# jshi31/T2ONet

Hardware: AMD Instinct MI355X
Metric: images/sec (train step: episode forward + END select + L1 + backward + gradient all-reduce + Adam, bs=64/GPU, 256x256 fp32) (higher is better)
Workload: dtype f32; 1 GPU; BASELINE.json configs[2]: full T2ONet episode/L1 train step (train_seq2seqL1.py:74-88), bs=64 per GPU, 256x256 fp32, FiveK-shaped synthetic batch, random-init weights; global_batch=64, parallelism=dp1: batch shards, one flat fp32 gradient all-reduce (22.2 M floats) per step, world_size=1

## Files before the change

include/t2onet_hip.h:

```cpp
#ifndef T2ONET_HIP_H
#define T2ONET_HIP_H

#include <stddef.h>

#ifdef __cplusplus
extern "C" {
#endif

#define T2O_OK 0
#define T2O_EINVAL 1
#define T2O_EUNSUPPORTED 2
#define T2O_EWORKSPACE 3
#define T2O_ELAUNCH 4

#define T2O_OP_IDENTITY (-1)
#define T2O_MAX_PARAM 24

int t2o_abi_version(void);
const char* t2o_last_error(void);
const char* t2o_source_digest(void);

int t2o_op_num_params(int op);

size_t t2o_workspace_bytes(int B, int H, int W);

int t2o_op_fwd(int op, const float* img, const float* param, int param_stride,
               const float* mask, int mask_ch, float* out, int B, int H, int W, void* stream);

int t2o_op_bwd(int op, const float* img, const float* param, int param_stride,
               const float* mask, int mask_ch, const float* gout,
               float* gimg, float* gparam, int gparam_stride,
               void* workspace, size_t workspace_bytes, int B, int H, int W, void* stream);

int t2o_apply_fwd(const int* op_id, const float* img, const float* param, int param_stride,
                  const float* mask, int mask_ch, float* out, int B, int H, int W, void* stream);
int t2o_apply_bwd(const int* op_id, const float* img, const float* param, int param_stride,
                  const float* mask, int mask_ch, const float* gout,
                  float* gimg, float* gparam, int gparam_stride,
                  void* workspace, size_t workspace_bytes, int B, int H, int W, void* stream);

int t2o_l1_fwd(const float* pred, const float* target, float* loss, size_t n,
               void* workspace, size_t workspace_bytes, void* stream);
int t2o_l1_bwd(const float* pred, const float* target, const float* gloss, float* gpred,
               size_t n, void* stream);

int t2o_end_select_l1_fwd(const float* const* imgs, int T, const long long* first, const float* target, float* loss, int B,
                          size_t row, void* workspace, size_t workspace_bytes, void* stream);
int t2o_end_select_l1_bwd(const float* const* imgs, float* const* gimgs, int T, const long long* first, const float* target,
                          const float* gloss, int B, size_t row, void* stream);

int t2o_op_fwd_l1(int op, const float* img, const float* param, int param_stride,
                  const float* mask, int mask_ch, const float* target, float* out, float* loss,
                  void* workspace, size_t workspace_bytes, int B, int H, int W, void* stream);
int t2o_op_bwd_l1(int op, const float* img, const float* param, int param_stride,
                  const float* mask, int mask_ch, const float* target, const float* gloss,
                  float* gimg, float* gparam, int gparam_stride,
                  void* workspace, size_t workspace_bytes, int B, int H, int W, void* stream);

int t2o_sequence_fwd(const int* ops, int K, const float* img, const float* params,
                     const float* target, float* acts, float* loss,
                     void* workspace, size_t workspace_bytes, int B, int H, int W, void* stream);
int t2o_sequence_bwd(const int* ops, int K, const float* img, const float* params,
                     const float* target, const float* acts, const float* gloss,
                     float* gimg, float* gparams, float* gbuf,
                     void* workspace, size_t workspace_bytes, int B, int H, int W, void* stream);

int t2o_fused_sequence_buffers(const int* ops, int K);
int t2o_fused_sequence_fwd(const int* ops, int K, const float* img, const float* params,
                           const float* target, float* out, float* loss, float* seg_bufs,
                           void* workspace, size_t workspace_bytes, int B, int H, int W, void* stream);
int t2o_fused_sequence_bwd(const int* ops, int K, const float* img, const float* params,
                           const float* target, const float* gloss, const float* gout,
                           float* gimg, float* gparams, const float* seg_bufs, float* gbuf,
                           void* workspace, size_t workspace_bytes, int B, int H, int W, void* stream);

int t2o_fused_sequence_l1_value_grad(const int* ops, int K, const float* img, const float* params,
                                     const float* target, const float* gloss, float* out, float* loss,
                                     float* gimg, float* gparams, float* seg_bufs, float* gbuf,
                                     void* workspace, size_t workspace_bytes, int B, int H, int W, void* stream);

int t2o_fused_sequence_prepare(const int* ops, int K);
int t2o_jit_set_cache_dir(const char* dir);
int t2o_jit_specialisations(void);

size_t t2o_candidates_workspace_bytes(int C, int H, int W);
int t2o_op_candidates_l1(int op, const float* img, const float* target, const float* params, int C,
                         int param_stride, float* loss, void* workspace, size_t workspace_bytes,
                         int H, int W, void* stream);

size_t t2o_candidates_multi_workspace_bytes(int J, int C, int H, int W);
int t2o_op_candidates_multi_l1(const int* ops, const int* img_index, int J, const float* imgs, int n_img,
                               const float* target, const float* params, int C, int param_stride, float* loss,
                               void* workspace, size_t workspace_bytes, int H, int W, void* stream);

size_t t2o_fit_multi_workspace_bytes(int J, int H, int W);
int t2o_fit_multi_l1_adam(const int* ops, const int* img_index, const int* target_index, int J, const float* imgs,
                          int n_img, const float* targets, int n_target, float* params, float* dist, void* workspace,
                          size_t workspace_bytes, int H, int W, int steps, double lr, double beta1, double beta2,
                          double eps, int check_every, double tol, void* stream);

size_t t2o_candidates_multi_masked_workspace_bytes(int J, int C, int H, int W);
int t2o_op_candidates_multi_l1_masked(const int* ops, const int* img_index, const int* mask_index, int J,
                                      const float* imgs, int n_img, const unsigned char* masks, int n_mask,
                                      const float* target, const float* params, int C, int param_stride, float* loss,
                                      void* workspace, size_t workspace_bytes, int H, int W, void* stream);
size_t t2o_fit_multi_masked_workspace_bytes(int J, int H, int W);
int t2o_fit_multi_l1_adam_masked(const int* ops, const int* img_index, const int* target_index, const int* mask_index,
                                 int J, const float* imgs, int n_img, const float* targets, int n_target,
                                 const unsigned char* masks, int n_mask, float* params, float* dist, void* workspace,
                                 size_t workspace_bytes, int H, int W, int steps, double lr, double beta1, double beta2,
                                 double eps, int check_every, double tol, void* stream);

size_t t2o_ssim_workspace_bytes(int B, int C, int H, int W);
int t2o_ssim_fwd(const float* img1, const float* img2, float* out,
                 void* workspace, size_t workspace_bytes, int B, int C, int H, int W, void* stream);
int t2o_ssim_bwd(const float* img1, const float* img2, const float* gout, float* g1, float* g2,
                 int B, int C, int H, int W, void* stream);

int t2o_attn_fwd(const float* q, const float* ctx, float* attn, float* mix,
                 int B, int L, int D, void* stream);
int t2o_attn_bwd(const float* q, const float* ctx, const float* attn, const float* gmix,
                 const float* gattn, float* gq, float* gctx, int B, int L, int D, void* stream);

int t2o_choose_op(const float* logp, float* op_mask, const float* u, float explore_prob, long long* pred_op, int* exec_op,
                  int B, int n_cls, void* stream);

size_t t2o_bn_workspace_bytes(int N, int C);
int t2o_bn_relu_fwd(const float* x, const float* res, const float* weight, const float* bias,
                    float* running_mean, float* running_var, float* save_mean, float* save_invstd, float* out,
                    float momentum, float eps, void* workspace, size_t workspace_bytes,
                    int N, int C, int HW, void* stream);
int t2o_bn_relu_bwd(const float* x, const float* y, const float* dy, const float* weight, const float* bias,
// ... 287 lines not shown
```

t2onet_amd/_lib.py:

```python
import ctypes
import os

import torch

_HERE = os.path.dirname(os.path.abspath(__file__))
LIB_PATH = os.path.join(_HERE, 'lib', 'libt2onet_hip.so')

c_f = ctypes.POINTER(ctypes.c_float)
c_i = ctypes.POINTER(ctypes.c_int)
_P = ctypes.c_void_p
_I = ctypes.c_int
_Z = ctypes.c_size_t
_F = ctypes.c_float
_D = ctypes.c_double

SIGNATURES = {
    't2o_abi_version': (_I, []),
    't2o_last_error': (ctypes.c_char_p, []),
    't2o_source_digest': (ctypes.c_char_p, []),
    't2o_op_num_params': (_I, [_I]),
    't2o_workspace_bytes': (_Z, [_I, _I, _I]),
    't2o_op_fwd': (_I, [_I, _P, _P, _I, _P, _I, _P, _I, _I, _I, _P]),
    't2o_op_bwd': (_I, [_I, _P, _P, _I, _P, _I, _P, _P, _P, _I, _P, _Z, _I, _I, _I, _P]),
    't2o_apply_fwd': (_I, [_P, _P, _P, _I, _P, _I, _P, _I, _I, _I, _P]),
    't2o_apply_bwd': (_I, [_P, _P, _P, _I, _P, _I, _P, _P, _P, _I, _P, _Z, _I, _I, _I, _P]),
    't2o_l1_fwd': (_I, [_P, _P, _P, _Z, _P, _Z, _P]),
    't2o_l1_bwd': (_I, [_P, _P, _P, _P, _Z, _P]),
    't2o_op_fwd_l1': (_I, [_I, _P, _P, _I, _P, _I, _P, _P, _P, _P, _Z, _I, _I, _I, _P]),
    't2o_op_bwd_l1': (_I, [_I, _P, _P, _I, _P, _I, _P, _P, _P, _P, _I, _P, _Z, _I, _I, _I, _P]),
    't2o_sequence_fwd': (_I, [_P, _I, _P, _P, _P, _P, _P, _P, _Z, _I, _I, _I, _P]),
    't2o_sequence_bwd': (_I, [_P, _I, _P, _P, _P, _P, _P, _P, _P, _P, _P, _Z, _I, _I, _I, _P]),
    't2o_fused_sequence_buffers': (_I, [_P, _I]),
    't2o_fused_sequence_fwd': (_I, [_P, _I, _P, _P, _P, _P, _P, _P, _P, _Z, _I, _I, _I, _P]),
    't2o_fused_sequence_bwd': (_I, [_P, _I, _P, _P, _P, _P, _P, _P, _P, _P, _P, _P, _Z, _I, _I, _I, _P]),
    't2o_fused_sequence_l1_value_grad': (_I, [_P, _I, _P, _P, _P, _P, _P, _P, _P, _P, _P, _P, _P, _Z, _I, _I, _I, _P]),
    't2o_candidates_workspace_bytes': (_Z, [_I, _I, _I]),
    't2o_op_candidates_l1': (_I, [_I, _P, _P, _P, _I, _I, _P, _P, _Z, _I, _I, _P]),
    't2o_candidates_multi_workspace_bytes': (_Z, [_I, _I, _I, _I]),
    't2o_op_candidates_multi_l1': (_I, [c_i, c_i, _I, _P, _I, _P, _P, _I, _I, _P, _P, _Z, _I, _I, _P]),
    't2o_fit_multi_workspace_bytes': (_Z, [_I, _I, _I]),
    't2o_fit_multi_l1_adam': (_I, [c_i, c_i, c_i, _I, _P, _I, _P, _I, _P, _P, _P, _Z, _I, _I, _I, _D, _D, _D, _D, _I, _D, _P]),
    't2o_candidates_multi_masked_workspace_bytes': (_Z, [_I, _I, _I, _I]),
    't2o_op_candidates_multi_l1_masked': (_I, [c_i, c_i, c_i, _I, _P, _I, _P, _I, _P, _P, _I, _I, _P, _P, _Z, _I, _I, _P]),
    't2o_fit_multi_masked_workspace_bytes': (_Z, [_I, _I, _I]),
    't2o_fit_multi_l1_adam_masked': (_I, [c_i, c_i, c_i, c_i, _I, _P, _I, _P, _I, _P, _I, _P, _P, _P, _Z, _I, _I, _I, _D, _D, _D, _D, _I,
                                          _D, _P]),
    't2o_ssim_workspace_bytes': (_Z, [_I, _I, _I, _I]),
    't2o_ssim_fwd': (_I, [_P, _P, _P, _P, _Z, _I, _I, _I, _I, _P]),
    't2o_ssim_bwd': (_I, [_P, _P, _P, _P, _P, _I, _I, _I, _I, _P]),
    't2o_wino_fused_wgrad_supported': (_I, [_I, _I, _I, _I, _I]),
    't2o_wino_fused_wgrad_workspace_bytes': (_Z, [_I, _I, _I, _I, _I]),
    't2o_wino_fused_wgrad_nhwc': (_I, [_P, _P, _P, _P, _P, _Z, _I, _I, _I, _I, _I, _I, _P]),
    't2o_comm_available': (_I, []),
    't2o_comm_unique_id': (_I, [_P]),
    't2o_comm_init_rank': (_I, [_P, _I, _P, _I]),
    't2o_comm_destroy': (_I, [_P]),
    't2o_allreduce': (_I, [_P, _Z, _P, _P]),
    't2o_allreduce_mean': (_I, [_P, _Z, _P, _P]),
    't2o_choose_op': (_I, [_P, _P, _P, _F, _P, _P, _I, _I, _P]),
    't2o_attn_fwd': (_I, [_P, _P, _P, _P, _I, _I, _I, _P]),
    't2o_attn_bwd': (_I, [_P, _P, _P, _P, _P, _P, _P, _I, _I, _I, _P]),
    't2o_bn_workspace_bytes': (_Z, [_I, _I]),
    't2o_bn_relu_fwd': (_I, [_P, _P, _P, _P, _P, _P, _P, _P, _P, _F, _F, _P, _Z, _I, _I, _I, _P]),
    't2o_bn_relu_bwd': (_I, [_P, _P, _P, _P, _P, _P, _P, _P, _P, _P, _P, _I, _P, _Z, _I, _I, _I, _P]),
    't2o_bn_nhwc_workspace_bytes': (_Z, [_I, _I]),
    't2o_bn_relu_nhwc_fwd': (_I, [_P, _P, _P, _P, _P, _P, _P, _P, _P, _F, _F, _I, _P, _Z, _I, _I, _P]),
    't2o_bn_relu_nhwc_bwd': (_I, [_P, _P, _P, _P, _P, _P, _P, _P, _P, _P, _P, _I, _I, _P, _Z, _I, _I, _P]),
    't2o_bn_relu_nhwc_fwd_partials': (_I, [_P, _P, _P, _P, _P, _P, _P, _P, _P, _F, _F, _I, _P, _I, _P, _Z, _I, _I, _P]),
    't2o_param_heads_fwd': (_I, [_P, _P, _P, _P, _P, _P, _P, _P, _P, _F, _F, _F, _F, _I, _I, _P]),
    't2o_param_heads_bwd': (_I, [_P, _P, _P, _P, _P, _P, _P, _P, _P, _P, _P, _P, _P, _P, _P, _F, _F, _F, _F, _I, _I, _P]),
    't2o_param_heads_bwd_acc': (_I, [_P, _P, _P, _P, _P, _P, _P, _P, _P, _P, _P, _P, _P, _P, _P, _F, _F, _F, _F, _I, _I, _I, _P]),
    't2o_adam_step': (_I, [_P, _P, _P, _P, _Z, _F, _F, _F, _F, _I, _P]),
    't2o_graph_memsets_to_kernels': (_I, [_P, _P]),
    't2o_conv3x3_wgrad_workspace_bytes': (_Z, [_I, _I, _I, _I, _I]),
    't2o_conv3x3_wgrad_nhwc': (_I, [_P, _P, _P, _P, _Z, _I, _I, _I, _I, _I, _P]),
    't2o_conv3x3_fwd_workspace_bytes': (_Z, [_I, _I, _I, _I, _I]),
    't2o_conv3x3_fwd_nhwc': (_I, [_P, _P, _P, _P, _Z, _I, _I, _I, _I, _I, _P]),
    't2o_conv3x3_dgrad_workspace_bytes': (_Z, [_I, _I, _I, _I, _I]),
    't2o_conv3x3_dgrad_nhwc': (_I, [_P, _P, _P, _P, _Z, _I, _I, _I, _I, _I, _P]),
    't2o_conv_set_zero_region': (_I, [_I, _P, _Z]),
    't2o_conv3x3s2_fwd_workspace_bytes': (_Z, [_I, _I, _I, _I, _I]),
    't2o_conv3x3s2_fwd_nhwc': (_I, [_P, _P, _P, _P, _Z, _I, _I, _I, _I, _I, _P]),
    't2o_conv3x3_fwd_stats_rows': (_I, [_I, _I, _I, _I, _I]),
    't2o_conv3x3_fwd_stats_nhwc': (_I, [_P, _P, _P, _P, _P, _Z, _I, _I, _I, _I, _I, _I, _P]),
    't2o_stem_fwd_stats_rows': (_I, [_I, _I, _I]),
    't2o_stem_fwd_nhwc': (_I, [_P, _P, _P, _P, _I, _I, _I, _I, _P]),
    't2o_stem_wgrad_workspace_bytes': (_Z, [_I, _I, _I, _I]),
    't2o_stem_wgrad_nhwc': (_I, [_P, _P, _P, _P, _Z, _I, _I, _I, _I, _P]),
    't2o_conv3x3s2_wgrad_workspace_bytes': (_Z, [_I, _I, _I, _I, _I]),
    't2o_conv3x3s2_wgrad_nhwc': (_I, [_P, _P, _P, _P, _Z, _I, _I, _I, _I, _I, _P]),
    't2o_conv3x3s2_dgrad_workspace_bytes': (_Z, [_I, _I, _I, _I, _I]),
    't2o_conv3x3s2_dgrad_nhwc': (_I, [_P, _P, _P, _P, _Z, _I, _I, _I, _I, _I, _P]),
    't2o_bn_relu_nhwc_bwd_acc': (_I, [_P, _P, _P, _P, _P, _P, _P, _P, _P, _P, _P, _I, _I, _I, _P, _Z, _I, _I, _P]),
    't2o_bn_relu_nhwc_bwd_partials_acc': (_I, [_P, _P, _P, _P, _P, _P, _P, _P, _P, _I, _I, _P, _I, _P, _Z, _I, _I, _P]),
    't2o_conv3x3_wgrad_acc_nhwc': (_I, [_P, _P, _P, _P, _Z, _I, _I, _I, _I, _I, _I, _I, _P]),
    't2o_conv_weight_transform': (_I, [_P, _P, _I, _I, _I, _I, _P]),
    't2o_conv_weight_transform_batch': (_I, [_P, _P, _P, _P, _P, _P, _I, _P]),
    't2o_wino_weight_transform_batch': (_I, [_P, _P, _P, _P, _I, _P]),
    't2o_wino_weight_transform_chunked_batch': (_I, [_P, _P, _P, _P, _I, _P]),
    't2o_end_select_l1_fwd': (_I, [_P, _I, _P, _P, _P, _I, _Z, _P, _Z, _P]),
    't2o_end_select_l1_bwd': (_I, [_P, _P, _I, _P, _P, _P, _I, _Z, _P]),
    't2o_wino_padded_tiles': (_I, [_I, _I, _I]),
    't2o_wino_weight_transform': (_I, [_P, _P, _I, _I, _P]),
    't2o_gemm_nt_batched': (_I, [_P, _P, _P, _I, _I, _I, _I, _I, _P]),
    't2o_gemm': (_I, [_P, _P, _P, _I, _I, _I, _I, _I, _I, _I, _I, _I, _P]),
    't2o_colsum': (_I, [_P, _P, _I, _I, _I, _I, _P]),
    't2o_gemm_tn_splits': (_I, [_I, _I, _I, _I]),
    't2o_gemm_tn_batched': (_I, [_P, _P, _P, _I, _I, _I, _I, _I, _P]),
    't2o_gemm_tn_batched_ld': (_I, [_P, _P, _P, _I, _I, _I, _I, _I, _I, _I, _P]),
    't2o_wino_input_transform': (_I, [_P, _P, _I, _I, _I, _I, _P]),
    't2o_wino_input_transform_ld': (_I, [_P, _P, _I, _I, _I, _I, _I, _P]),
    't2o_wino_stats_rows': (_I, [_I, _I, _I, _I]),
    't2o_wino_output_transform': (_I, [_P, _P, _P, _P, _I, _I, _I, _I, _P]),
    't2o_wino_dy_transform': (_I, [_P, _P, _I, _I, _I, _I, _P]),
    't2o_wino_dy_transforms': (_I, [_P, _P, _P, _I, _I, _I, _I, _P]),
    't2o_wino_dy_transforms_ld': (_I, [_P, _P, _P, _I, _I, _I, _I, _I, _P]),
    't2o_wino_dy_transform_ld': (_I, [_P, _P, _I, _I, _I, _I, _I, _P]),
    't2o_wino_dw_transform': (_I, [_P, _P, _I, _I, _I, _I, _P]),
    't2o_conv3x3_dgrad_pre_nhwc': (_I, [_P, _P, _P, _P, _P, _Z, _I, _I, _I, _I, _I, _P]),
    't2o_conv3x3_dgrad_bnsums_rows': (_I, [_I, _I, _I, _I, _I]),
    't2o_wino_fused_supported': (_I, [_I, _I, _I, _I, _I]),
    't2o_wino_fused_stats_rows': (_I, [_I, _I, _I]),
    't2o_wino_u_chunked': (_I, [_P, _P, _I, _I, _P]),
    't2o_wino_fused_conv_nhwc': (_I, [_P, _P, _P, _P, _P, _P, _I, _I, _I, _I, _I, _P]),
    't2o_wino_fused_conv_bnsums_nhwc': (_I, [_P, _P, _P, _P, _P, _P, _P, _P, _P, _P, _I, _I, _I, _I, _I, _P]),
    't2o_conv3x3_dgrad_pre_bnsums_nhwc': (_I, [_P, _P, _P, _P, _P, _P, _P, _P, _P, _P, _Z, _I, _I, _I, _I, _I, _P]),
    't2o_conv3x3s2_dgrad_pre_nhwc': (_I, [_P, _P, _P, _P, _Z, _I, _I, _I, _I, _I, _P]),
    't2o_stem_fwd': (_I, [_P, _P, _P, _P, _I, _I, _I, _I, _I, _P]),
    't2o_stem_fwd_any': (_I, [_P, _P, _P, _P, _I, _I, _I, _I, _I, _P]),
    't2o_stem_wgrad': (_I, [_P, _P, _P, _P, _Z, _I, _I, _I, _I, _I, _I, _P]),
    't2o_stem_dgrad': (_I, [_P, _P, _P, _I, _I, _I, _I, _I, _I, _P]),
    't2o_conv1x1s2_fwd_nhwc': (_I, [_P, _P, _P, _I, _I, _I, _I, _I, _P]),
    't2o_conv1x1s2_dgrad_acc_nhwc': (_I, [_P, _P, _P, _I, _I, _I, _I, _I, _P]),
    't2o_conv1x1s2_wgrad_workspace_bytes': (_Z, [_I, _I, _I, _I, _I]),
    't2o_conv1x1s2_wgrad_nhwc': (_I, [_P, _P, _P, _P, _Z, _I, _I, _I, _I, _I, _I, _P]),
    't2o_fused_sequence_prepare': (_I, [_P, _I]),
    't2o_jit_set_cache_dir': (_I, [ctypes.c_char_p]),
    't2o_jit_specialisations': (_I, []),
    't2o_conv3x3_any_fwd_nhwc': (_I, [_P, _P, _P, _I, _I, _I, _I, _I, _I, _P]),
    't2o_conv3x3_any_dgrad_nhwc': (_I, [_P, _P, _P, _P, _I, _I, _I, _I, _I, _I, _P]),
    't2o_conv3x3_any_wgrad_workspace_bytes': (_Z, [_I, _I, _I, _I, _I, _I]),
    't2o_conv3x3_any_wgrad_nhwc': (_I, [_P, _P, _P, _P, _Z, _I, _I, _I, _I, _I, _I, _I, _P]),
    't2o_lstm_layer_fwd': (_I, [_P, _P, _P, _P, _P, _P, _P, _P, _P, _I, _I, _I, _I, _P]),
    't2o_lstm_layer_bwd': (_I, [_P, _P, _P, _P, _P, _P, _P, _P, _P, _P, _I, _I, _I, _I, _P]),
    't2o_bn_dual_nhwc_workspace_bytes': (_Z, [_I, _I]),
    't2o_bn_dual_relu_nhwc_fwd': (_I, [_P, _P, _I, _P] + [_P] * 13 + [_F, _F, _F, _F, _P, _Z, _I, _I, _P]),
    't2o_bn_dual_relu_nhwc_bwd_acc': (_I, [_P] * 18 + [_I, _P, _Z, _I, _I, _P]),
    't2o_image_feature_fwd': (_I, [_P, _P]),
    't2o_image_feature_bwd': (_I, [_P, _P]),
    't2o_decoder_step_fwd': (_I, [_P, _P]),
    't2o_decoder_step_bwd': (_I, [_P, _P]),
    't2o_resize_u8_to_f32': (_I, [_P, _P, _I, _I, _I, _P, _P]),
    't2o_f32_to_u8_hwc': (_I, [_P, _I, _I, _I, _P, _P]),
    't2o_replay_u8': (_I, [_P, _P, _P, _I, _P, _P]),
    't2o_replay_u8_masked': (_I, [_P, _P, _P, _P, _I, _P, _P, _P, _I, _P]),
    't2o_feather_weights': (_I, [_D, _P, _P]),
    't2o_feather_workspace_bytes': (_Z, [_P, _I]),
    't2o_feather_u8': (_I, [_P, _P, _P, _I, _P, _Z, _P]),
    't2o_eval_metrics_workspace_bytes': (_Z, [_I, _I, _I, _I]),
    't2o_eval_metrics': (_I, [_P, _P, _I, _P, _P, _P, _I, _P, _Z, _I, _I, _I, _I, _P]),
    't2o_end_select_var_mean_workspace_bytes': (_Z, [_Z]),
    't2o_end_select_var_mean': (_I, [_P, _P, _I, _I, _I, _Z, _P, _P, _Z, _P]),
    't2o_rle_union_u8': (_I, [_P, _P, _I, _I, _I, ctypes.c_longlong, _P, ctypes.c_longlong, _P]),
    't2o_mask_select': (_I, [_P, _P, _P, _P, _I, _I, _I, _I, _I, _P]),
}


class ImageFeatureArgs(ctypes.Structure):
    _fields_ = ([(n, _P) for n in ('fc_w', 'fc_b', 'bn_w', 'bn_b', 'running_mean', 'running_var', 'num_batches_tracked', 'pooled',
                                   'pooled_copy', 'fc_out', 'stats', 'feat', 'g_feat', 'd_fc', 'd_bn', 'd_pooled')]
                + [('momentum', _F), ('eps', _F), ('training', _I), ('B', _I), ('K', _I), ('D', _I)])


class DecoderStepArgs(ctypes.Structure):
    _fields_ = ([(n, _P) for n in ('emb', 'vis_w', 'vis_b', 'w_ih0', 'w_hh0', 'b_ih0', 'b_hh0', 'w_ih1', 'w_hh1', 'b_ih1', 'b_hh1',
                                   'lo_w', 'lo_b', 'out_w', 'out_b', 'prev_op', 'feat', 'h0', 'c0', 'h1', 'c1', 'enc', 'step_in',
                                   'feat_copy', 'hp0', 'hp1', 'prev_op_copy', 'gates0', 'gates1', 'h0n', 'c0n', 'h1n', 'c1n', 'attn', 'mix', 'ctx', 'logp',
                                   'g_logp', 'g_ctx', 'g_h0n', 'g_c0n', 'g_h1n', 'g_c1n', 'd_logits', 'd_lin', 'd_gates1',
                                   'd_gates0', 'd_step_in', 'd_vis', 'd_ctx', 'd_mix', 'd_qa', 'd_q', 'd_x1', 'd_feat', 'd_h0',
                                   'd_c0', 'd_h1', 'd_c1', 'd_enc')]
                + [(n, _I) for n in ('B', 'L', 'D', 'E', 'V')])

_lib = None

# ... 42 lines not shown
```

t2onet_amd/csrc/t2o_block_programs.h:

```cpp
#pragma once
#ifndef __HIPCC_RTC__
#include <stddef.h>
#include <stdint.h>
#endif

#include "t2o_pixel_math.h"

namespace t2o {

constexpr int kThreads = 256;
constexpr int kRedSlots = 24;

constexpr int kTileW = 64;
constexpr int kTileH = 16;
constexpr int kStripRows = 4;
constexpr int kStripWideCols = 248;
T2O_HD int strip_bwd_segments(int W) { return W <= 256 ? 1 : (W + kStripWideCols - 1) / kStripWideCols; }
constexpr int kFwdStripRows = 2;
constexpr int kRowStride = 72;
constexpr int kIntOff = 4;

struct OpArgs {
  const float* img;
  const float* param;
  const float* mask;
  const int* op_id;
  const float* gout;
  const float* target;
  const float* gloss;
  float* out;
  float* gimg;
  float* partials;
  float* loss_partials;
  int op;
  int param_stride;
  int mask_ch;
  int B, H, W;
  int iters;
  int nblk_max;
  float inv_n;
};

T2O_HD size_t plane_off(const OpArgs& a, int b, int c) { return ((size_t)b * 3 + c) * (size_t)a.H * a.W; }

T2O_HD float mask_at(const OpArgs& a, int b, int c, size_t px) {
  const int mc = a.mask_ch == 3 ? c : 0;
  return a.mask[((size_t)b * a.mask_ch + mc) * (size_t)a.H * a.W + px];
}

template <int V>
T2O_HD void load_vec(const float* p, float (&r)[V]) {
#if defined(__HIP_DEVICE_COMPILE__)
  if constexpr (V == 4) {
    const float4 t = *reinterpret_cast<const float4*>(p);
    r[0] = t.x; r[1] = t.y; r[2] = t.z; r[3] = t.w;
    return;
  }
#endif
  T2O_UNROLL
  for (int i = 0; i < V; ++i) r[i] = p[i];
}

template <int V>
T2O_HD void store_vec(float* p, const float (&r)[V]) {
#if defined(__HIP_DEVICE_COMPILE__)
  if constexpr (V == 4) {
    *reinterpret_cast<float4*>(p) = make_float4(r[0], r[1], r[2], r[3]);
    return;
  }
#endif
  T2O_UNROLL
  for (int i = 0; i < V; ++i) p[i] = r[i];
}

T2O_HD float sign_of(float d) { return d > 0.0f ? 1.0f : (d < 0.0f ? -1.0f : 0.0f); }

constexpr int kTabStride = 64;
constexpr int kTabK = 0, kTabP = 24, kTabSum = 51, kTabScale = 54, kTabRsum = 57;

T2O_HD void curve_table_build(const float* p, bool color, float* t) {
  for (int c = 0; c < 3; ++c) {
    const float* row = color ? p + c * kCurveSteps : p;
    float s = 0.0f, run = 0.0f;
    for (int i = 0; i < kCurveSteps; ++i) {
      t[kTabK + c * kCurveSteps + i] = row[i];
      t[kTabP + c * (kCurveSteps + 1) + i] = run;
      run = run + (1.0f / kCurveSteps) * row[i];
      s = s + row[i];
    }
    t[kTabP + c * (kCurveSteps + 1) + kCurveSteps] = run;
    s = s + 1e-10f;
    t[kTabSum + c] = s;
    t[kTabRsum + c] = 1.0f / s;
    t[kTabScale + c] = t[kTabRsum + c] * (float)kCurveSteps;
  }
}

T2O_HD void curve_locate(float x, int& i, float& frac, bool unit = false) {
  const float x8 = unit ? fminf(x * (float)kCurveSteps, (float)kCurveSteps - 0.5f)
                        : fminf(fmaxf(x * (float)kCurveSteps, 0.0f), (float)kCurveSteps - 0.5f);
  i = (int)x8;
  const float d = x - (float)i / kCurveSteps;
  frac = unit ? d : fminf(fmaxf(d, 0.0f), 1.0f / kCurveSteps);
}

T2O_HD float curve_lut_fwd(const float* t, bool color, int c, float x, bool unit = false) {
  const int cc = color ? c : 0;
  int i; float frac;
  curve_locate(x, i, frac, unit);
  const float total = t[kTabP + cc * (kCurveSteps + 1) + i] + frac * t[kTabK + cc * kCurveSteps + i];
  return color ? total * t[kTabScale + cc]
               : div_by(total * (float)kCurveSteps, t[kTabSum + cc], t[kTabRsum + cc]);
}

T2O_HD float curve_lut_bwd_1(const float* t, bool color, int c, float x, float g, float* red_row, bool first = false,
                             bool unit = false) {
  const int cc = color ? c : 0;
  const float* kk = t + kTabK + cc * kCurveSteps;
  int i; float frac;
  curve_locate(x, i, frac, unit);
  const float d = x - (float)i / kCurveSteps;
  float slope = (unit || (d >= 0.0f && d <= 1.0f / kCurveSteps)) ? kk[i] : 0.0f;
  if (d == 0.0f && i > 0) slope += kk[i - 1];
  curve_bins_accumulate(x, g, red_row, first);
  return g * t[kTabScale + cc] * slope;
}

struct SampleView {
  const float* x;
  const float* g;
  const float* m;
  float* o;
  const float* t;
  unsigned hw;
  unsigned mstride;
};

template <int V, bool MASKED, bool L1>
T2O_HD float pointwise_fwd_thread(const OpArgs& a, int op, int b, int blk, int tid) {
  const unsigned hw = (unsigned)a.H * (unsigned)a.W;
  const unsigned groups = hw / V;
  const size_t sb = (size_t)b * 3 * hw;
  SampleView s;
  s.x = a.img + sb;
  s.o = a.out + sb;
  s.t = L1 ? a.target + sb : nullptr;
  s.m = MASKED ? a.mask + (size_t)b * a.mask_ch * hw : nullptr;
  s.mstride = (MASKED && a.mask_ch == 3) ? hw : 0u;
  const float* prow = a.param ? a.param + (size_t)b * a.param_stride : nullptr;
  Curve cv;
  if (op == OP_COLOR || op == OP_TONE) curve_load(cv, prow, op == OP_COLOR);
  float p0[1] = {(op >= 0 && prow) ? prow[0] : 0.0f};
  float l1 = 0.0f;
  for (int it = 0; it < a.iters; ++it) {
    const unsigned g = ((unsigned)blk * a.iters + it) * kThreads + tid;
    if (g >= groups) break;
    const unsigned px = g * V;
    float x[3][V], o[3][V], mk[3][V];
    T2O_UNROLL
    for (int c = 0; c < 3; ++c) {
      load_vec<V>(s.x + c * hw + px, x[c]);
      if (MASKED && (c == 0 || s.mstride)) load_vec<V>(s.m + c * s.mstride + px, mk[c]);
    }
    T2O_UNROLL
    for (int i = 0; i < V; ++i) {
      Rgb xi = {{x[0][i], x[1][i], x[2][i]}};
      if (op == OP_IDENTITY) {
        o[0][i] = xi.c[0]; o[1][i] = xi.c[1]; o[2][i] = xi.c[2];
      } else {
        const Rgb r = pointwise_fwd(op, xi, p0, cv);
        T2O_UNROLL
        for (int c = 0; c < 3; ++c) {
          float z = r.c[c];
          if (MASKED) z = blend(z, xi.c[c], s.mstride ? mk[c][i] : mk[0][i]);
          o[c][i] = clamp01(z);
        }
      }
    }
    T2O_UNROLL
    for (int c = 0; c < 3; ++c) store_vec<V>(s.o + c * hw + px, o[c]);
    if (L1) {
      T2O_UNROLL
      for (int c = 0; c < 3; ++c) {
        float t[V];
        load_vec<V>(s.t + c * hw + px, t);
        T2O_UNROLL
        for (int i = 0; i < V; ++i) l1 += fabsf(o[c][i] - t[i]);
      }
    }
  }
  return l1;
}

template <int V, bool MASKED, bool L1>
T2O_HD void pointwise_bwd_thread(const OpArgs& a, int op, int b, int blk, int tid, float (&red)[kRedSlots], const float* tab) {
  const unsigned hw = (unsigned)a.H * (unsigned)a.W;
  const unsigned groups = hw / V;
  const size_t sb = (size_t)b * 3 * hw;
  SampleView s;
  s.x = a.img + sb;
  s.g = (L1 ? a.target : a.gout) + sb;
  s.o = a.gimg ? a.gimg + sb : nullptr;
  s.m = MASKED ? a.mask + (size_t)b * a.mask_ch * hw : nullptr;
  s.mstride = (MASKED && a.mask_ch == 3) ? hw : 0u;
  const float* prow = a.param ? a.param + (size_t)b * a.param_stride : nullptr;
  Curve cv;
  float p0[1] = {(op >= 0 && prow) ? prow[0] : 0.0f};
  const float gs = L1 ? a.gloss[0] * a.inv_n : 0.0f;
  for (int it = 0; it < a.iters; ++it) {
    const unsigned g = ((unsigned)blk * a.iters + it) * kThreads + tid;
    if (g >= groups) break;
    const unsigned px = g * V;
    float x[3][V], gg[3][V], gx[3][V], mk[3][V];
    T2O_UNROLL
    for (int c = 0; c < 3; ++c) {
      load_vec<V>(s.x + c * hw + px, x[c]);
      load_vec<V>(s.g + c * hw + px, gg[c]);
      if (MASKED && (c == 0 || s.mstride)) load_vec<V>(s.m + c * s.mstride + px, mk[c]);
    }
    if (op == OP_TONE || op == OP_COLOR) {
      const bool color = op == OP_COLOR;
      float dep = 0.0f;
      T2O_UNROLL
      for (int i = 0; i < V; ++i) {
        T2O_UNROLL
        for (int c = 0; c < 3; ++c) {
          const float xv = T2O_CHAIN(x[c][i], dep);
          const float r = curve_lut_fwd(tab, color, c, xv);
          const float m = MASKED ? (s.mstride ? mk[c][i] : mk[0][i]) : 1.0f;
          const float z = MASKED ? blend(r, xv, m) : r;
          const float gz = L1 ? sign_of(clamp01(z) - gg[c][i]) * gs : gg[c][i];
          const float dz = (z >= 0.0f && z <= 1.0f) ? gz : 0.0f;
          const int kc = color ? c : 0;
          const float gi = curve_lut_bwd_1(tab, color, c, xv, MASKED ? dz * m : dz, red + kc * kCurveSteps);
          gx[c][i] = MASKED ? gi + dz * (1.0f - m) : gi;
          dep = gx[c][i];
          T2O_UNROLL
          for (int j = 0; j < kCurveSteps; ++j) T2O_KEEP(red[kc * kCurveSteps + j]);
        }
      }
    } else {
    T2O_UNROLL
    for (int i = 0; i < V; ++i) {
      Rgb xi = {{x[0][i], x[1][i], x[2][i]}};
      if (op == OP_IDENTITY) {
        T2O_UNROLL
        for (int c = 0; c < 3; ++c) gx[c][i] = L1 ? sign_of(xi.c[c] - gg[c][i]) * gs : gg[c][i];
        continue;
      }
      Rgb go, gpass;
      if (!MASKED && !L1 && !clamp_can_act(op, xi)) {
        go.c[0] = gg[0][i]; go.c[1] = gg[1][i]; go.c[2] = gg[2][i];
        const Rgb gi = pointwise_bwd(op, xi, p0, cv, go, red);
        T2O_UNROLL
        for (int c = 0; c < 3; ++c) gx[c][i] = gi.c[c];
        continue;
      }
      const Rgb r = pointwise_fwd(op, xi, p0, cv);
      T2O_UNROLL
      for (int c = 0; c < 3; ++c) {
        const float m = MASKED ? (s.mstride ? mk[c][i] : mk[0][i]) : 1.0f;
        const float z = MASKED ? blend(r.c[c], xi.c[c], m) : r.c[c];
        const float gz = L1 ? sign_of(clamp01(z) - gg[c][i]) * gs : gg[c][i];
        const float dz = (z >= 0.0f && z <= 1.0f) ? gz : 0.0f;
        go.c[c] = MASKED ? dz * m : dz;
        gpass.c[c] = MASKED ? dz * (1.0f - m) : 0.0f;
      }
      const Rgb gi = pointwise_bwd(op, xi, p0, cv, go, red);
      T2O_UNROLL
      for (int c = 0; c < 3; ++c) gx[c][i] = gi.c[c] + gpass.c[c];
    }
    }
    if (s.o) {
      T2O_UNROLL
      for (int c = 0; c < 3; ++c) store_vec<V>(s.o + c * hw + px, gx[c]);
    }
  }
}

T2O_HD int tile_rows(int halo) { return kTileH + 2 * halo; }
T2O_HD int tile_floats(int halo) { return tile_rows(halo) * kRowStride; }

template <int V, int HALO>
T2O_HD void tile_load(const float* src, unsigned hw, int planes, int H, int W, int y0, int x0, float* lds, int tid) {
  constexpr int rows = kTileH + 2 * HALO;
  constexpr int plane_floats = rows * kRowStride;
  if (V == 4) {
    constexpr int per_plane = rows * (kTileW / 4);
    for (int i = tid; i < planes * per_plane; i += kThreads) {
      const int c = i / per_plane, rem = i % per_plane;
      const int r = rem / (kTileW / 4), q = rem % (kTileW / 4);
      const int gy = y0 - HALO + r, gx = x0 + 4 * q;
      float v[4] = {0.0f, 0.0f, 0.0f, 0.0f};
      if (gy >= 0 && gy < H && gx < W) load_vec<4>(src + ((unsigned)c * hw + (unsigned)gy * (unsigned)W + (unsigned)gx), v);
      store_vec<4>(lds + c * plane_floats + r * kRowStride + kIntOff + 4 * q, v);
    }
    constexpr int hper = rows * 2 * HALO;
    for (int i = tid; i < planes * hper; i += kThreads) {
      const int c = i / hper, rem = i % hper;
      const int r = rem / (2 * HALO), k = rem % (2 * HALO);
      const int j = k < HALO ? k - HALO : kTileW + (k - HALO);
      const int gy = y0 - HALO + r, gx = x0 + j;
      float v = 0.0f;
      if (gy >= 0 && gy < H && gx >= 0 && gx < W) v = src[(unsigned)c * hw + (unsigned)gy * (unsigned)W + (unsigned)gx];
      lds[c * plane_floats + r * kRowStride + kIntOff + j] = v;
    }
  } else {
    constexpr int cols = kTileW + 2 * HALO;
    constexpr int per_plane = rows * cols;
    for (int i = tid; i < planes * per_plane; i += kThreads) {
      const int c = i / per_plane, rem = i % per_plane;
      const int r = rem / cols, j = rem % cols - HALO;
      const int gy = y0 - HALO + r, gx = x0 + j;
      float v = 0.0f;
      if (gy >= 0 && gy < H && gx >= 0 && gx < W) v = src[(unsigned)c * hw + (unsigned)gy * (unsigned)W + (unsigned)gx];
      lds[c * plane_floats + r * kRowStride + kIntOff + j] = v;
    }
  }
}

T2O_HD float tile_at(const float* lds, int halo, int c, int r, int j) {
  return lds[c * tile_floats(halo) + (r + halo) * kRowStride + kIntOff + j];
}

T2O_HD void tile_origin(const OpArgs& a, int tile, int& y0, int& x0) {
  const int tiles_x = (a.W + kTileW - 1) / kTileW;
  y0 = (tile / tiles_x) * kTileH;
  x0 = (tile % tiles_x) * kTileW;
}
T2O_HD int sharp_num_tiles(int H, int W) {
  return ((W + kTileW - 1) / kTileW) * ((H + kTileH - 1) / kTileH);
}

T2O_HD int sharp_fwd_lds_floats() { return 3 * tile_floats(1); }

template <int V>
T2O_HD void sharp_fwd_phase_load(const OpArgs& a, int b, int tile, int tid, float* lds) {
  int y0, x0;
  tile_origin(a, tile, y0, x0);
  tile_load<V, 1>(a.img + plane_off(a, b, 0), (unsigned)a.H * (unsigned)a.W, 3, a.H, a.W, y0, x0, lds, tid);
}

T2O_HD void tile_quad(const float* lds, int halo, int c, int r, int j, float (&q)[4]) {
  load_vec<4>(lds + c * tile_floats(halo) + (r + halo) * kRowStride + kIntOff + j, q);
}

struct Sides { float L, R; };
T2O_HD Sides quad_sides(const float* lds, int halo, int c, int r, int j0, const float (&ce)[4]) {
  Sides s;
#if defined(__HIP_DEVICE_COMPILE__)
  const float l = __builtin_bit_cast(float, __builtin_amdgcn_update_dpp(0, __builtin_bit_cast(int, ce[3]), 0x111, 0xF, 0xF, true));
  const float rr = __builtin_bit_cast(float, __builtin_amdgcn_update_dpp(0, __builtin_bit_cast(int, ce[0]), 0x101, 0xF, 0xF, true));
  const float e = tile_at(lds, halo, c, r, j0 == 0 ? -1 : kTileW);
  s.L = j0 == 0 ? e : l;
  s.R = j0 == kTileW - 4 ? e : rr;
#else
// ... 95 lines not shown
      const bool in = n == 4 ? quad_in : (row_in && x0 + j0 + i >= 0 && x0 + j0 + i < a.W);
      const float left = i == 0 ? L : ce[i > 0 ? i - 1 : 0], right = i == n - 1 ? R : ce[i < 3 ? i + 1 : 3];
      const float d = sharp_delta(ce[i], up[i], left, right, dn[i]);
      const float m = a.mask_ch ? mq[i] : 1.0f;
      float z = ce[i] + p * d;
      if (a.mask_ch) z = blend(z, ce[i], m);
      const float gz = a.target ? sign_of(clamp01(z) - gq[i]) * gs : gq[i];
      dz[i] = (in && z >= 0.0f && z <= 1.0f) ? gz : 0.0f;
      if (interior) red0 += dz[i] * m * d;
    }
  }
  float* dst = G + c * tile_floats(1) + (r + 1) * kRowStride + kIntOff + j0;
  if (n == 4) store_vec<4>(dst, dz); else dst[0] = dz[0];
}

template <int V>
T2O_HD void sharp_bwd_phase_dz(const OpArgs& a, int b, int tile, int tid, float* lds, float& red0) {
  int y0, x0;
  tile_origin(a, tile, y0, x0);
  const float p = a.param[(size_t)b * a.param_stride];
  const float gs = a.target ? a.gloss[0] * a.inv_n : 0.0f;
  const int rows = kTileH + 2;
  if (V == 4) {
    const int per = rows * (kTileW / 4);
    for (int i = tid; i < 3 * per; i += kThreads) {
      const int c = i / per, rem = i % per;
      sharp_dz_quad(a, p, gs, y0, x0, c, rem / (kTileW / 4) - 1, 4 * (rem % (kTileW / 4)), 4, lds, red0);
    }
    for (int i = tid; i < 3 * rows * 2; i += kThreads) {
      const int c = i / (rows * 2), rem = i % (rows * 2);
      sharp_dz_quad(a, p, gs, y0, x0, c, rem / 2 - 1, (rem % 2) ? kTileW : -1, 1, lds, red0);
    }
  } else {
    const int cols = kTileW + 2, per = rows * cols;
    for (int i = tid; i < 3 * per; i += kThreads) {
      const int c = i / per, rem = i % per;
      sharp_dz_quad(a, p, gs, y0, x0, c, rem / cols - 1, rem % cols - 1, 1, lds, red0);
    }
  }
}

template <int V>
T2O_HD void sharp_bwd_phase_out(const OpArgs& a, int b, int tile, int tid, const float* lds) {
  int y0, x0;
  tile_origin(a, tile, y0, x0);
  const int ty = tid / (kTileW / 4), tx = tid % (kTileW / 4);
  const int gy = y0 + ty, gx0 = x0 + 4 * tx;
  const bool live = gy < a.H && gx0 < a.W && a.gimg;
  const float p = a.param[(size_t)b * a.param_stride];
  const float* G = lds + sharp_bwd_g_off();
  const float* M = lds + sharp_bwd_m_off();
  T2O_UNROLL
  for (int c = 0; c < 3; ++c) {
    const int mc = a.mask_ch == 3 ? c : 0;
    float up[4], ce[4], dn[4], o[4], pass[4];
    tile_quad(G, 1, c, ty - 1, 4 * tx, up);
    tile_quad(G, 1, c, ty, 4 * tx, ce);
    tile_quad(G, 1, c, ty + 1, 4 * tx, dn);
    const Sides sg = quad_sides(G, 1, c, ty, 4 * tx, ce);
    float L = sg.L, R = sg.R;
    T2O_UNROLL
    for (int i = 0; i < 4; ++i) pass[i] = 0.0f;
    if (a.mask_ch) {
      float mu[4], mcq[4], md[4];
      tile_quad(M, 1, mc, ty - 1, 4 * tx, mu);
      tile_quad(M, 1, mc, ty, 4 * tx, mcq);
      tile_quad(M, 1, mc, ty + 1, 4 * tx, md);
      const Sides sm = quad_sides(M, 1, mc, ty, 4 * tx, mcq);
      L *= sm.L;
      R *= sm.R;
      T2O_UNROLL
      for (int i = 0; i < 4; ++i) {
        pass[i] = ce[i] * (1.0f - mcq[i]);
        up[i] *= mu[i]; ce[i] *= mcq[i]; dn[i] *= md[i];
      }
    }
    T2O_UNROLL
    for (int i = 0; i < 4; ++i) {
      const float left = i == 0 ? L : ce[i > 0 ? i - 1 : 0], right = i == 3 ? R : ce[i < 3 ? i + 1 : 3];
      o[i] = pass[i] + (ce[i] + p * sharp_delta(ce[i], up[i], left, right, dn[i]));
    }
    if (!live) continue;
    float* dst = a.gimg + plane_off(a, b, c) + (size_t)gy * a.W + gx0;
    if (V == 4) store_vec<4>(dst, o);
    else for (int i = 0; i < 4 && gx0 + i < a.W; ++i) dst[i] = o[i];
  }
}

constexpr int kMaxChain = 8;
constexpr int kAccStride = 65;

struct ChainArgs {
  const float* img;
  const float* params;
  const float* gout;
  const float* target;
  const float* gloss;
  float* out;
  float* gimg;
  float* partials;
  float* loss_partials;
  int ops[kMaxChain];
  int src[kMaxChain];
  int slot_off[kMaxChain + 1];
  int bin_off[kMaxChain + 1];
  int K, B, H, W, iters, nblk;
  int param_stride, gparam_stride;
  float inv_n;
};

T2O_HD bool is_curve(int op) { return op == OP_COLOR || op == OP_TONE; }

T2O_HD void chain_build_table(const ChainArgs& a, int b, int k, float* tab) {
  float* t = tab + k * kTabStride;
  const float* p = a.params + ((size_t)a.src[k] * a.B + b) * a.param_stride;
  const int op = a.ops[k];
  if (!is_curve(op)) { t[0] = p[0]; return; }
  curve_table_build(p, op == OP_COLOR, t);
}

T2O_HD Rgb chain_op_fwd(int op, const Rgb& x, const float* t, bool unit = false) {
  Rgb o;
  switch (op) {
    case OP_BRIGHTNESS: return brightness_fwd(x, t[0]);
    case OP_CONTRAST:   return contrast_fwd(x, t[0]);
    case OP_SATURATION: return saturation_fwd(x, t[0]);
    case OP_COLOR:
    case OP_TONE:
      T2O_UNROLL
      for (int c = 0; c < 3; ++c) o.c[c] = curve_lut_fwd(t, op == OP_COLOR, c, x.c[c], unit);
      return o;
    case OP_WHITE: o.c[0] = o.c[1] = o.c[2] = 1.0f; return o;
    default: return x;
  }
}

template <bool COLOR>
T2O_HD Rgb chain_curve_bwd(const Rgb& x, const float* t, const Rgb& dz, float* red, bool first, bool unit = false) {
  Rgb gx;
  T2O_UNROLL
  for (int c = 0; c < 3; ++c) {
    constexpr int kOne = COLOR ? 1 : 0;
    const int cc = c * kOne;
    gx.c[c] = curve_lut_bwd_1(t, COLOR, c, x.c[c], dz.c[c], red + cc * kCurveSteps, first && (COLOR || c == 0), unit);
  }
  return gx;
}

T2O_HD float chain_slot_value(const ChainArgs& a, int s, const float* bsum) { return bsum[s]; }

T2O_HD Rgb chain_scalar_bwd(int op, const Rgb& x, const float* t, const Rgb& dz, float* red) {
  Curve unused;
  float p0[1] = {t[0]};
  return pointwise_bwd(op, x, p0, unused, dz, red);
}

template <int V, bool L1>
T2O_HD float chain_fwd_thread(const ChainArgs& a, int b, int blk, int tid, const float* tab) {
  const unsigned hw = (unsigned)a.H * (unsigned)a.W;
  const unsigned groups = hw / V;
  const size_t sb = (size_t)b * 3 * hw;
  const float* xin = a.img + sb;
  float* o = a.out + sb;
  float l1 = 0.0f;
  for (int it = 0; it < a.iters; ++it) {
    const unsigned g = ((unsigned)blk * a.iters + it) * kThreads + tid;
// ... 692 lines not shown
```

t2onet_amd/csrc/t2o_kernels.hip:

```cpp
#include <hip/hip_runtime.h>
#include <stdio.h>
#include <stdlib.h>
#include <string.h>

#include <type_traits>

#include "../../include/t2onet_hip.h"
#include "t2o_block_programs.h"
#include "t2o_chain_kernels.h"
#include "t2o_jit.h"

using namespace t2o;

namespace {

thread_local char g_err[256] = "";

int fail(int code, const char* msg) {
  snprintf(g_err, sizeof(g_err), "%s", msg);
  return code;
}

}
namespace t2o { int set_error(int code, const char* msg) { return fail(code, msg); } }
namespace {

template <int OP, int V, bool MASKED, bool L1>
__global__ __launch_bounds__(kThreads) void k_point_fwd(OpArgs a, int nblk) {
  int b, blk;
  wg_coords(nblk, b, blk);
  const int op = (OP == OP_DYNAMIC) ? a.op_id[b] : OP;
  if (OP == OP_DYNAMIC && op == OP_SHARPNESS) return;
  float l1 = 0.0f;
  if (OP == OP_DYNAMIC) {
    switch (op) {
#define T2O_CASE(K) case K: l1 = pointwise_fwd_thread<V, MASKED, L1>(a, K, b, blk, threadIdx.x); break;
      T2O_CASE(OP_BRIGHTNESS) T2O_CASE(OP_CONTRAST) T2O_CASE(OP_SATURATION) T2O_CASE(OP_COLOR)
      T2O_CASE(OP_TONE) T2O_CASE(OP_WHITE)
#undef T2O_CASE
      default: l1 = pointwise_fwd_thread<V, MASKED, L1>(a, OP_IDENTITY, b, blk, threadIdx.x); break;
    }
  } else {
    l1 = pointwise_fwd_thread<V, MASKED, L1>(a, OP, b, blk, threadIdx.x);
  }
  if (L1) block_reduce_store1(l1, a.loss_partials + (size_t)b * a.nblk_max + blk);
}

template <int OP, int V, bool MASKED, bool L1>
__global__ __launch_bounds__(kThreads) void k_point_bwd(OpArgs a, int nblk) {
  int b, blk;
  wg_coords(nblk, b, blk);
  const int op = (OP == OP_DYNAMIC) ? a.op_id[b] : OP;
  if (OP == OP_DYNAMIC && op == OP_SHARPNESS) return;
  float red[kRedSlots];
#pragma unroll
  for (int i = 0; i < kRedSlots; ++i) red[i] = 0.0f;
  __shared__ float tab[kTabStride];
  if (OP == OP_COLOR || OP == OP_TONE || OP == OP_DYNAMIC) {
    if ((op == OP_COLOR || op == OP_TONE) && threadIdx.x == 0)
      curve_table_build(a.param + (size_t)b * a.param_stride, op == OP_COLOR, tab);
    __syncthreads();
  }
  if (OP == OP_DYNAMIC) {
    switch (op) {
#define T2O_CASE(K) case K: pointwise_bwd_thread<V, MASKED, L1>(a, K, b, blk, threadIdx.x, red, tab); break;
      T2O_CASE(OP_BRIGHTNESS) T2O_CASE(OP_CONTRAST) T2O_CASE(OP_SATURATION) T2O_CASE(OP_COLOR)
      T2O_CASE(OP_TONE) T2O_CASE(OP_WHITE)
#undef T2O_CASE
      default: pointwise_bwd_thread<V, MASKED, L1>(a, OP_IDENTITY, b, blk, threadIdx.x, red, tab); break;
    }
  } else {
    pointwise_bwd_thread<V, MASKED, L1>(a, OP, b, blk, threadIdx.x, red, tab);
  }
  if (op == OP_IDENTITY || op == OP_WHITE) return;
  block_reduce_store(red, nred_of(op), a.partials + ((size_t)b * a.nblk_max + blk) * kRedSlots);
}

template <bool DYN, int V>
__global__ __launch_bounds__(kThreads) void k_sharp_fwd(OpArgs a, int tiles) {
  extern __shared__ __attribute__((aligned(16))) float lds[];
  int b, tile;
  wg_coords(tiles, b, tile);
  if (DYN && a.op_id[b] != OP_SHARPNESS) return;
  sharp_fwd_phase_load<V>(a, b, tile, threadIdx.x, lds);
  __syncthreads();
  const float l1 = sharp_fwd_phase_compute<V>(a, b, tile, threadIdx.x, lds);
  if (a.target) block_reduce_store1(l1, a.loss_partials + (size_t)b * a.nblk_max + tile);
}


__device__ __forceinline__ float dpp_wave_shr1(float v) {
  return __builtin_bit_cast(float, __builtin_amdgcn_update_dpp(0, __builtin_bit_cast(int, v), 0x138, 0xF, 0xF, true));
}
__device__ __forceinline__ float dpp_wave_shl1(float v) {
  return __builtin_bit_cast(float, __builtin_amdgcn_update_dpp(0, __builtin_bit_cast(int, v), 0x130, 0xF, 0xF, true));
}

template <bool DYN, bool WIDE, int ROWS>
__global__ __launch_bounds__(kThreads) void k_sharp_fwd_strip(OpArgs a, int nblk, int nseg) {
  int b, blk;
  wg_coords(nblk, b, blk);
  if (DYN && a.op_id[b] != OP_SHARPNESS) return;
  const int lane = threadIdx.x & 63, wave = threadIdx.x >> 6;
  const int y0 = (blk / nseg) * (4 * ROWS) + wave * ROWS, gx0 = (blk % nseg) * 256 + 4 * lane;
  const bool col_live = gx0 < a.W;
  const unsigned hw = (unsigned)a.H * (unsigned)a.W;
  const float p = a.param[(size_t)b * a.param_stride];
  const bool ext_l = WIDE && lane == 0 && gx0 > 0 && col_live, ext_r = WIDE && lane == 63 && gx0 + 4 < a.W;
  float l1 = 0.0f;
#pragma unroll 1
  for (int c = 0; c < 3; ++c) {
    const float* xp = a.img + ((size_t)b * 3 + c) * hw;
    float xr[ROWS + 2][4], tg[ROWS][4];
#pragma unroll
    for (int k = 0; k < ROWS + 2; ++k) {
      const int y = y0 - 1 + k;
      xr[k][0] = xr[k][1] = xr[k][2] = xr[k][3] = 0.0f;
      if (col_live && y >= 0 && y < a.H) load_vec<4>(xp + (unsigned)y * (unsigned)a.W + (unsigned)gx0, xr[k]);
    }
    if (a.target) {
#pragma unroll
      for (int k = 0; k < ROWS; ++k) {
        const int y = y0 + k;
        tg[k][0] = tg[k][1] = tg[k][2] = tg[k][3] = 0.0f;
        if (col_live && y < a.H) load_vec<4>(a.target + ((size_t)b * 3 + c) * hw + (unsigned)y * (unsigned)a.W + (unsigned)gx0, tg[k]);
      }
    }
#pragma unroll
    for (int k = 0; k < ROWS; ++k) {
      const int y = y0 + k;
      const bool live = col_live && y < a.H;
      const float* ce = xr[k + 1];
      float L = dpp_wave_shr1(ce[3]), R = dpp_wave_shl1(ce[0]);
      if (ext_l && live) L = xp[(unsigned)y * (unsigned)a.W + (unsigned)gx0 - 1];
      if (ext_r && live) R = xp[(unsigned)y * (unsigned)a.W + (unsigned)gx0 + 4];
      float o[4];
#pragma unroll
      for (int i = 0; i < 4; ++i) {
        const float left = i == 0 ? L : ce[i > 0 ? i - 1 : 0], right = i == 3 ? R : ce[i < 3 ? i + 1 : 3];
        o[i] = ce[i] + p * sharp_delta(ce[i], xr[k][i], left, right, xr[k + 2][i]);
      }
      if (!live) continue;
      const unsigned off = (unsigned)y * (unsigned)a.W + (unsigned)gx0;
      if (a.mask_ch) {
        float m[4];
        load_vec<4>(a.mask + ((size_t)b * a.mask_ch + (a.mask_ch == 3 ? c : 0)) * hw + off, m);
#pragma unroll
        for (int i = 0; i < 4; ++i) o[i] = blend(o[i], ce[i], m[i]);
      }
#pragma unroll
      for (int i = 0; i < 4; ++i) o[i] = clamp01(o[i]);
      store_vec<4>(a.out + ((size_t)b * 3 + c) * hw + off, o);
      if (a.target) {
#pragma unroll
        for (int i = 0; i < 4; ++i) l1 += fabsf(o[i] - tg[k][i]);
      }
    }
  }
  if (a.target) block_reduce_store1(l1, a.loss_partials + (size_t)b * a.nblk_max + blk);
}


template <bool DYN, bool WIDE, bool MASKED, bool VAL = false>
__global__ __launch_bounds__(kThreads) void k_sharp_bwd_strip(OpArgs a, int nblk, int nseg) {
  int b, blk;
  wg_coords(nblk, b, blk);
  if (DYN && a.op_id[b] != OP_SHARPNESS) return;
  const int lane = threadIdx.x & 63, wave = threadIdx.x >> 6;
  const int y0 = (blk / nseg) * (4 * kStripRows) + wave * kStripRows;
  const int gx0 = WIDE ? (blk % nseg) * kStripWideCols - 4 + 4 * lane : 4 * lane;
  const bool col_live = gx0 >= 0 && gx0 < a.W;
  const bool own = !WIDE || (lane >= 1 && lane <= 62);
  const unsigned hw = (unsigned)a.H * (unsigned)a.W;
  const float p = a.param[(size_t)b * a.param_stride];
  const float gs = a.target ? a.gloss[0] * a.inv_n : 0.0f;
  float red0 = 0.0f;
  float l1 = 0.0f;
#pragma unroll 1
  for (int c = 0; c < 3; ++c) {
    const float* xp = a.img + ((size_t)b * 3 + c) * hw;
    const float* gp = (a.target ? a.target : a.gout) + ((size_t)b * 3 + c) * hw;
    const float* mp = MASKED ? a.mask + ((size_t)b * a.mask_ch + (a.mask_ch == 3 ? c : 0)) * hw : nullptr;
    float xr[kStripRows + 4][4], g[kStripRows + 2][4], mk[MASKED ? kStripRows + 2 : 1][4], pass[MASKED ? kStripRows : 1][4];
#pragma unroll
    for (int k = 0; k < kStripRows + 4; ++k) {
      const int y = y0 - 2 + k;
      xr[k][0] = xr[k][1] = xr[k][2] = xr[k][3] = 0.0f;
      if (col_live && y >= 0 && y < a.H) load_vec<4>(xp + (unsigned)y * (unsigned)a.W + (unsigned)gx0, xr[k]);
    }
#pragma unroll
    for (int k = 0; k < kStripRows + 2; ++k) {
      const int y = y0 - 1 + k;
      g[k][0] = g[k][1] = g[k][2] = g[k][3] = 0.0f;
      if (MASKED) mk[k][0] = mk[k][1] = mk[k][2] = mk[k][3] = 0.0f;
      if (col_live && y >= 0 && y < a.H) {
        load_vec<4>(gp + (unsigned)y * (unsigned)a.W + (unsigned)gx0, g[k]);
        if (MASKED) load_vec<4>(mp + (unsigned)y * (unsigned)a.W + (unsigned)gx0, mk[k]);
      }
    }
#pragma unroll
    for (int k = 0; k < kStripRows + 2; ++k) {
      const int y = y0 - 1 + k;
      const bool in = col_live && y >= 0 && y < a.H;
      const float* ce = xr[k + 1];
      const float L = dpp_wave_shr1(ce[3]), R = dpp_wave_shl1(ce[0]);
      const bool mine = VAL && k >= 1 && k <= kStripRows && own && in;
      float oz[VAL ? 4 : 1];
#pragma unroll
      for (int i = 0; i < 4; ++i) {
        const float left = i == 0 ? L : ce[i > 0 ? i - 1 : 0], right = i == 3 ? R : ce[i < 3 ? i + 1 : 3];
        const float d = sharp_delta(ce[i], xr[k][i], left, right, xr[k + 2][i]);
        const float m = MASKED ? mk[k][i] : 1.0f;
        float z = ce[i] + p * d;
        if (MASKED) z = blend(z, ce[i], m);
        if constexpr (VAL) {
          oz[i] = clamp01(z);
          if (mine) l1 += fabsf(oz[i] - g[k][i]);
        }
        const float gz = a.target ? sign_of(clamp01(z) - g[k][i]) * gs : g[k][i];
        const float dz = (in && z >= 0.0f && z <= 1.0f) ? gz : 0.0f;
        g[k][i] = MASKED ? dz * m : dz;
        if (MASKED && k >= 1 && k <= kStripRows) pass[k - 1][i] = dz * (1.0f - m);
        if (k >= 1 && k <= kStripRows && own) red0 += dz * m * d;
      }
      if constexpr (VAL) {
        if (a.out && mine) store_vec<4>(a.out + ((size_t)b * 3 + c) * hw + (unsigned)y * (unsigned)a.W + (unsigned)gx0, oz);
      }
    }
#pragma unroll
    for (int k = 1; k <= kStripRows; ++k) {
      const int y = y0 - 1 + k;
      const float* ce = g[k];
      const float L = dpp_wave_shr1(ce[3]), R = dpp_wave_shl1(ce[0]);
      float o[4];
#pragma unroll
      for (int i = 0; i < 4; ++i) {
        const float left = i == 0 ? L : ce[i > 0 ? i - 1 : 0], right = i == 3 ? R : ce[i < 3 ? i + 1 : 3];
        o[i] = ce[i] + p * sharp_delta(ce[i], g[k - 1][i], left, right, g[k + 1][i]);
        if (MASKED) o[i] = pass[k - 1][i] + o[i];
      }
      if (a.gimg && own && col_live && y < a.H)
        store_vec<4>(a.gimg + ((size_t)b * 3 + c) * hw + (unsigned)y * (unsigned)a.W + (unsigned)gx0, o);
    }
  }
  block_reduce_store1(red0, a.partials + ((size_t)b * a.nblk_max + blk) * kRedSlots);
  if constexpr (VAL) {
    __syncthreads();
    block_reduce_store1(l1, a.loss_partials + (size_t)b * a.nblk_max + blk);
  }
}

template <bool DYN, int V>
__global__ __launch_bounds__(kThreads) void k_sharp_bwd(OpArgs a, int tiles) {
  extern __shared__ __attribute__((aligned(16))) float lds[];
  int b, tile;
  wg_coords(tiles, b, tile);
  if (DYN && a.op_id[b] != OP_SHARPNESS) return;
  sharp_bwd_phase_load<V>(a, b, tile, threadIdx.x, lds);
  __syncthreads();
  float red0 = 0.0f;
  sharp_bwd_phase_dz<V>(a, b, tile, threadIdx.x, lds, red0);
  __syncthreads();
  sharp_bwd_phase_out<V>(a, b, tile, threadIdx.x, lds);
  block_reduce_store1(red0, a.partials + ((size_t)b * a.nblk_max + tile) * kRedSlots);
}

template <int V, bool L1>
__global__ __launch_bounds__(kThreads) void k_chain_fwd(ChainArgs a) {
  __shared__ float tab[kMaxChain * kTabStride];
  int b, blk;
  wg_coords(a.nblk, b, blk);
  if ((int)threadIdx.x < a.K) chain_build_table(a, b, threadIdx.x, tab);
  __syncthreads();
  const float l1 = chain_fwd_thread<V, L1>(a, b, blk, threadIdx.x, tab);
  if (L1) block_reduce_store1(l1, a.loss_partials + (size_t)b * a.nblk + blk);
}

template <int V, bool L1, class SEQ>
__global__ __launch_bounds__(kThreads) void k_chain_fwd_static(ChainArgs a) { chain_fwd_static_body<V, L1, SEQ>(a); }

template <int V, bool L1>
__global__ __launch_bounds__(kThreads) void k_chain_bwd(ChainArgs a) {
  extern __shared__ __attribute__((aligned(16))) float lds[];
  __shared__ float tab[kMaxChain * kTabStride];
  __shared__ float bsum[kMaxChainBins];
  int b, blk;
  wg_coords(a.nblk, b, blk);
  const int S = a.slot_off[kMaxChain], NB = a.bin_off[kMaxChain];
  for (int i = threadIdx.x; i < NB * kAccStride; i += kThreads) lds[i] = 0.0f;
  if ((int)threadIdx.x < a.K) chain_build_table(a, b, threadIdx.x, tab);
  __syncthreads();
  LdsAcc acc{lds};
  const float l1 = chain_bwd_thread<V, L1>(a, b, blk, threadIdx.x, tab, lds + NB * kAccStride, acc);
  if (L1 && a.loss_partials) block_reduce_store1(l1, a.loss_partials + (size_t)b * a.nblk + blk);
  __syncthreads();
  for (int s = threadIdx.x; s < NB; s += kThreads) {
    float sum = 0.0f;
    for (int q = 0; q < kThreads / 4; ++q) sum += lds[s * kAccStride + q];
    bsum[s] = sum;
  }
  __syncthreads();
  for (int s = threadIdx.x; s < S; s += kThreads)
    a.partials[((size_t)b * a.nblk + blk) * S + s] = chain_slot_value(a, s, bsum);
}

template <bool L1, class SEQ, bool SV_LDS, int MINW, bool VAL = false>
__global__ __launch_bounds__(kThreads, MINW) void k_chain_bwd_static(ChainArgs a) { chain_bwd_static_body<L1, SEQ, SV_LDS, VAL>(a); }

__global__ __launch_bounds__(kThreads) void k_chain_finalize(ChainArgs a, float* gparams) {
  __shared__ float part[8][kMaxChainSlots];
  __shared__ float sums[kMaxChainSlots];
  const int b = blockIdx.x;
  const int S = a.slot_off[kMaxChain];
  for (int w = threadIdx.x; w < S * 8; w += kThreads) {
    const int s = w % S, lane8 = w / S;
    float acc = 0.0f;
    for (int k = lane8; k < a.nblk; k += 8) acc += a.partials[((size_t)b * a.nblk + k) * S + s];
    part[lane8][s] = acc;
  }
  __syncthreads();
  for (int s = threadIdx.x; s < S; s += kThreads) {
    float v = 0.0f;
#pragma unroll
    for (int j = 0; j < 8; ++j) v += part[j][s];
    sums[s] = v;
// ... 120 lines not shown
  for (int it = 0; it < iters; ++it) {
    const size_t g = ((size_t)blockIdx.x * iters + it) * kThreads + threadIdx.x;
    if (g * V >= n) break;
    float p[V], t[V];
    load_vec<V>(pred + g * V, p);
    load_vec<V>(target + g * V, t);
#pragma unroll
    for (int i = 0; i < V; ++i) acc += fabsf(p[i] - t[i]);
  }
  block_reduce_store1(acc, partial + blockIdx.x);
}

__global__ __launch_bounds__(kThreads) void k_l1_finalize(const float* partial, int nblk, float inv_n, float* loss) {
  float acc = 0.0f;
  for (int k = threadIdx.x; k < nblk; k += kThreads) acc += partial[k];
  __shared__ float out1;
  block_reduce_store1(acc, &out1);
  __syncthreads();
  if (threadIdx.x == 0) loss[0] = out1 * inv_n;
}

template <int V>
__global__ __launch_bounds__(kThreads) void k_l1_bwd(const float* pred, const float* target, const float* gloss,
                                                     float* gpred, size_t n, float inv_n, int iters) {
  const float gs = gloss[0] * inv_n;
  for (int it = 0; it < iters; ++it) {
    const size_t g = ((size_t)blockIdx.x * iters + it) * kThreads + threadIdx.x;
    if (g * V >= n) break;
    float p[V], t[V], o[V];
    load_vec<V>(pred + g * V, p);
    load_vec<V>(target + g * V, t);
#pragma unroll
    for (int i = 0; i < V; ++i) o[i] = sign_of(p[i] - t[i]) * gs;
    store_vec<V>(gpred + g * V, o);
  }
}

struct EndSelArgs {
  const float* img[8];
  float* gimg[8];
  int T;
};

__device__ __forceinline__ const float* end_sel_src(const EndSelArgs& s, int f) {
  const float* p = s.img[0];
#pragma unroll
  for (int t = 1; t < 8; ++t) p = (f == t) ? s.img[t] : p;
  return p;
}

template <int V>
__global__ __launch_bounds__(kThreads) void k_end_l1_fwd(EndSelArgs s, const long long* first, const float* target, float* partial,
                                                         size_t n, size_t row, int iters) {
  float acc = 0.0f;
  for (int it = 0; it < iters; ++it) {
    const size_t g = ((size_t)blockIdx.x * iters + it) * kThreads + threadIdx.x;
    if (g * V >= n) break;
    const int f = (int)first[(g * V) / row];
    float p[V], t[V];
    load_vec<V>(end_sel_src(s, f) + g * V, p);
    load_vec<V>(target + g * V, t);
#pragma unroll
    for (int i = 0; i < V; ++i) acc += fabsf(p[i] - t[i]);
  }
  block_reduce_store1(acc, partial + blockIdx.x);
}

template <int V>
__global__ __launch_bounds__(kThreads) void k_end_l1_bwd(EndSelArgs s, const long long* first, const float* target, const float* gloss,
                                                         size_t n, size_t row, float inv_n, int iters) {
  const float gs = gloss[0] * inv_n;
  for (int it = 0; it < iters; ++it) {
    const size_t g = ((size_t)blockIdx.x * iters + it) * kThreads + threadIdx.x;
    if (g * V >= n) break;
    const int f = (int)first[(g * V) / row];
    float p[V], t[V], o[V], z[V];
    load_vec<V>(end_sel_src(s, f) + g * V, p);
    load_vec<V>(target + g * V, t);
#pragma unroll
    for (int i = 0; i < V; ++i) { o[i] = sign_of(p[i] - t[i]) * gs; z[i] = 0.0f; }
#pragma unroll
    for (int k = 0; k < 8; ++k)
      if (k < s.T) store_vec<V>(s.gimg[k] + g * V, f == k ? o : z);
  }
}

__global__ __launch_bounds__(kThreads) void k_ssim_fwd(SsimArgs s) {
  extern __shared__ __attribute__((aligned(16))) float lds[];
  int plane, tile;
  wg_coords(s.tiles, plane, tile);
  ssim_phase_load(s, plane, tile, threadIdx.x, lds);
  __syncthreads();
  ssim_phase_rows(s, threadIdx.x, lds);
  __syncthreads();
  const float v = ssim_phase_cols(s, tile, threadIdx.x, lds);
  block_reduce_store1(v, s.partials + (size_t)plane * s.tiles + tile);
}

__global__ __launch_bounds__(kThreads) void k_ssim_finalize(const float* partials, int per_sample, float inv, float* out) {
  float acc = 0.0f;
  for (int k = threadIdx.x; k < per_sample; k += kThreads) acc += partials[(size_t)blockIdx.x * per_sample + k];
  __shared__ float out1;
  block_reduce_store1(acc, &out1);
  __syncthreads();
  if (threadIdx.x == 0) out[blockIdx.x] = out1 * inv;
}

__global__ __launch_bounds__(kThreads) void k_ssim_bwd(SsimBwdArgs s) {
  __shared__ __attribute__((aligned(16))) float lds[kSsimBD + 4 * kSsimBMid * kSsimBMidStride];
  int plane, tile;
  wg_coords(s.tiles, plane, tile);
  ssim_bwd_phase_load(s, plane, tile, threadIdx.x, lds);
  __syncthreads();
  ssim_bwd_phase_rows(s, threadIdx.x, lds);
  __syncthreads();
  ssim_bwd_phase_deriv(s, plane, tile, threadIdx.x, lds);
  __syncthreads();
  ssim_bwd_phase_drows(s, threadIdx.x, lds);
  __syncthreads();
  ssim_bwd_phase_out(s, plane, tile, threadIdx.x, lds);
}

__global__ __launch_bounds__(kThreads) void k_candidates_l1(CandArgs a) {
  __shared__ float tab[kCandPerBlock * kTabStride];
  __shared__ float wsum[kCandPerBlock][kThreads / 64];
  const int blk = blockIdx.x % a.nblk, group = blockIdx.x / a.nblk;
  const int c0 = group * kCandPerBlock;
  if ((int)threadIdx.x < kCandPerBlock && c0 + (int)threadIdx.x < a.C)
    cand_build_table(a, c0 + threadIdx.x, tab + threadIdx.x * kTabStride);
  float x[3][kCandPix], tg[3][kCandPix];
  const int npx = cand_load(a, blk, threadIdx.x, x, tg);
  __syncthreads();
  for (int j = 0; j < kCandPerBlock; ++j) {
    if (c0 + j >= a.C) break;
    const float s = wave_sum(cand_eval(a, tab + j * kTabStride, x, tg, npx));
    if ((threadIdx.x & 63) == 0) wsum[j][threadIdx.x >> 6] = s;
  }
  __syncthreads();
  if ((int)threadIdx.x < kCandPerBlock && c0 + (int)threadIdx.x < a.C) {
    const int j = threadIdx.x;
    a.partials[(size_t)(c0 + j) * a.nblk + blk] = ((wsum[j][0] + wsum[j][1]) + wsum[j][2]) + wsum[j][3];
  }
}

constexpr int kMaxCandJobs = 64;
struct MultiCandArgs {
  const float* imgs;
  const float* target;
  const float* params;
  float* partials;
  int op[kMaxCandJobs];
  int img_index[kMaxCandJobs];
  int C, param_stride, H, W, nblk;
};

struct MultiCandMaskArgs : MultiCandArgs {
  const unsigned char* masks;
  int mask_index[kMaxCandJobs];
};

template <bool MASKED>
__global__ __launch_bounds__(kThreads) void k_candidates_multi_l1(typename std::conditional<MASKED, MultiCandMaskArgs, MultiCandArgs>::type m) {
  __shared__ float tab[kCandPerBlock * kTabStride];
  __shared__ float wsum[kCandPerBlock][kThreads / 64];
  const int job = blockIdx.y;
  CandArgs a;
// ... 244 lines not shown
  const float* cb = ctx + (size_t)b * L * D;
  const float* gm = gmix + (size_t)b * D;
  for (int l = wave; l < L; l += kThreads / 64) {
    float part = 0.0f;
    for (int e = lane; e < D; e += 64) part += gm[e] * cb[(size_t)l * D + e];
    const float s = wave_sum(part);
    if (lane == 0) ga[l] = s + (gattn ? gattn[(size_t)b * L + l] : 0.0f);
  }
  if ((int)threadIdx.x < L) pr[threadIdx.x] = attn[(size_t)b * L + threadIdx.x];
  __syncthreads();
  float dot = 0.0f;
  for (int l = 0; l < L; ++l) dot += pr[l] * ga[l];
  if ((int)threadIdx.x < L) gs[threadIdx.x] = pr[threadIdx.x] * (ga[threadIdx.x] - dot);
  __syncthreads();
  for (int e = threadIdx.x; e < D; e += kThreads) {
    const float qe = qb[e], ge = gm[e];
    float acc = 0.0f;
    for (int l = 0; l < L; ++l) {
      acc += gs[l] * cb[(size_t)l * D + e];
      gctx[((size_t)b * L + l) * D + e] = pr[l] * ge + gs[l] * qe;
    }
    gq[(size_t)b * D + e] = acc;
  }
}

int env_int(const char* name, int dflt) {
  const char* s = getenv(name);
  return s ? atoi(s) : dflt;
}

Geometry launch_geometry(int B, int H, int W) {
  constexpr int forced = 0;
  return t2o::geometry(B, H, W, forced);
}

size_t ws_block_rows(const Geometry& g, int B, int H, int W) {
  int vec, iters, nblk;
  chain_geometry(B, H, W, 0, vec, iters, nblk, 1);
  return (size_t)(g.nblk_max > nblk ? g.nblk_max : nblk);
}
size_t ws_partials_floats(const Geometry& g, int B, int H, int W) { return (size_t)B * ws_block_rows(g, B, H, W) * kMaxChainSlots; }
size_t ws_loss_floats(const Geometry& g, int B, int H, int W) { return (size_t)B * ws_block_rows(g, B, H, W); }

int check_launch(const char* what) {
  const hipError_t e = hipGetLastError();
  if (e != hipSuccess) {
    snprintf(g_err, sizeof(g_err), "%s: %s", what, hipGetErrorString(e));
    return T2O_ELAUNCH;
  }
  return T2O_OK;
}

bool op_supported(int op) { return op == OP_IDENTITY || (op >= 0 && op <= 7 && op != OP_INPAINT); }

#define T2O_POINT_OPS(KERNEL, V, M, L)                                                        \
  switch (op) {                                                                             \
    case OP_IDENTITY:   KERNEL<OP_IDENTITY, V, M, L><<<grid, kThreads, 0, st>>>(a, nblk); break;   \
    case OP_BRIGHTNESS: KERNEL<OP_BRIGHTNESS, V, M, L><<<grid, kThreads, 0, st>>>(a, nblk); break; \
    case OP_CONTRAST:   KERNEL<OP_CONTRAST, V, M, L><<<grid, kThreads, 0, st>>>(a, nblk); break;   \
    case OP_SATURATION: KERNEL<OP_SATURATION, V, M, L><<<grid, kThreads, 0, st>>>(a, nblk); break; \
    case OP_COLOR:      KERNEL<OP_COLOR, V, M, L><<<grid, kThreads, 0, st>>>(a, nblk); break;      \
    case OP_TONE:       KERNEL<OP_TONE, V, M, L><<<grid, kThreads, 0, st>>>(a, nblk); break;       \
    case OP_WHITE:      KERNEL<OP_WHITE, V, M, L><<<grid, kThreads, 0, st>>>(a, nblk); break;      \
    case OP_DYNAMIC:    KERNEL<OP_DYNAMIC, V, M, L><<<grid, kThreads, 0, st>>>(a, nblk); break;    \
    default: break;                                                                         \
  }
#define T2O_POINT_CASES(KERNEL, V)                                    \
  if (masked) {                                                       \
    if (l1) { T2O_POINT_OPS(KERNEL, V, true, true) } else { T2O_POINT_OPS(KERNEL, V, true, false) }   \
  } else {                                                            \
    if (l1) { T2O_POINT_OPS(KERNEL, V, false, true) } else { T2O_POINT_OPS(KERNEL, V, false, false) } \
  }

void launch_point_fwd(const OpArgs& a, const Geometry& g, hipStream_t st) {
  const int op = a.op, nblk = g.nblk_point;
  const bool masked = a.mask_ch != 0, l1 = a.target != nullptr;
  const unsigned grid = (unsigned)a.B * nblk;
  if (g.vec == 4) { T2O_POINT_CASES(k_point_fwd, 4) } else { T2O_POINT_CASES(k_point_fwd, 1) }
}
void launch_point_bwd(const OpArgs& a, const Geometry& g, hipStream_t st) {
  const int op = a.op, nblk = g.nblk_point;
  const bool masked = a.mask_ch != 0, l1 = a.target != nullptr;
  const unsigned grid = (unsigned)a.B * nblk;
  if (g.vec == 4) { T2O_POINT_CASES(k_point_bwd, 4) } else { T2O_POINT_CASES(k_point_bwd, 1) }
}
bool sharp_uses_strips(const Geometry& g) {
  constexpr int mode = 1;
  return mode && g.vec_tile == 4;
}
bool sharp_bwd_uses_strips(const OpArgs&, const Geometry& g) { return sharp_uses_strips(g); }
int sharp_fwd_blocks(const OpArgs&, const Geometry& g) { return sharp_uses_strips(g) ? g.nblk_strip_fwd : g.nblk_sharp; }
int sharp_bwd_blocks(const OpArgs& a, const Geometry& g) { return sharp_bwd_uses_strips(a, g) ? g.nblk_strip_bwd : g.nblk_sharp; }

void launch_sharp_fwd(const OpArgs& a, const Geometry& g, hipStream_t st) {
  if (sharp_uses_strips(g)) {
    const int nseg = (a.W + 255) / 256, nblk = sharp_fwd_blocks(a, g);
    const unsigned grid = (unsigned)a.B * nblk;
    const bool dyn = a.op == OP_DYNAMIC;
    constexpr int R = kFwdStripRows;
    if (nseg > 1) { if (dyn) k_sharp_fwd_strip<true, true, R><<<grid, kThreads, 0, st>>>(a, nblk, nseg); else k_sharp_fwd_strip<false, true, R><<<grid, kThreads, 0, st>>>(a, nblk, nseg); }
    else          { if (dyn) k_sharp_fwd_strip<true, false, R><<<grid, kThreads, 0, st>>>(a, nblk, nseg); else k_sharp_fwd_strip<false, false, R><<<grid, kThreads, 0, st>>>(a, nblk, nseg); }
    return;
  }
  const unsigned grid = (unsigned)a.B * g.nblk_sharp;
  const size_t lds = sizeof(float) * sharp_fwd_lds_floats();
  const bool dyn = a.op == OP_DYNAMIC;
  if (g.vec_tile == 4) {
    if (dyn) k_sharp_fwd<true, 4><<<grid, kThreads, lds, st>>>(a, g.nblk_sharp);
    else k_sharp_fwd<false, 4><<<grid, kThreads, lds, st>>>(a, g.nblk_sharp);
  } else {
    if (dyn) k_sharp_fwd<true, 1><<<grid, kThreads, lds, st>>>(a, g.nblk_sharp);
    else k_sharp_fwd<false, 1><<<grid, kThreads, lds, st>>>(a, g.nblk_sharp);
  }
}
void launch_sharp_bwd(const OpArgs& a, const Geometry& g, hipStream_t st) {
  if (sharp_bwd_uses_strips(a, g)) {
    const int nseg = strip_bwd_segments(a.W), nblk = g.nblk_strip_bwd;
    const unsigned grid = (unsigned)a.B * nblk;
    const bool dyn = a.op == OP_DYNAMIC;
    if (a.loss_partials) {
      if (nseg > 1) k_sharp_bwd_strip<false, true, false, true><<<grid, kThreads, 0, st>>>(a, nblk, nseg);
      else k_sharp_bwd_strip<false, false, false, true><<<grid, kThreads, 0, st>>>(a, nblk, nseg);
      return;
    }
#define T2O_BWD_STRIP(D, Wd) \
    { if (a.mask_ch) k_sharp_bwd_strip<D, Wd, true><<<grid, kThreads, 0, st>>>(a, nblk, nseg); \
      else k_sharp_bwd_strip<D, Wd, false><<<grid, kThreads, 0, st>>>(a, nblk, nseg); }
    if (nseg > 1) { if (dyn) T2O_BWD_STRIP(true, true) else T2O_BWD_STRIP(false, true) }
    else          { if (dyn) T2O_BWD_STRIP(true, false) else T2O_BWD_STRIP(false, false) }
#undef T2O_BWD_STRIP
    return;
  }
  const unsigned grid = (unsigned)a.B * g.nblk_sharp;
  const size_t lds = sizeof(float) * sharp_bwd_lds_floats(a.mask_ch);
  const bool dyn = a.op == OP_DYNAMIC;
  if (g.vec_tile == 4) {
    if (dyn) k_sharp_bwd<true, 4><<<grid, kThreads, lds, st>>>(a, g.nblk_sharp);
    else k_sharp_bwd<false, 4><<<grid, kThreads, lds, st>>>(a, g.nblk_sharp);
  } else {
    if (dyn) k_sharp_bwd<true, 1><<<grid, kThreads, lds, st>>>(a, g.nblk_sharp);
    else k_sharp_bwd<false, 1><<<grid, kThreads, lds, st>>>(a, g.nblk_sharp);
  }
}

int check_common(int op, const int* op_id, const float* img, const float* param, int param_stride,
                 const float* mask, int mask_ch, int B, int H, int W) {
  if (B <= 0 || H <= 0 || W <= 0) return fail(T2O_EINVAL, "B, H, W must be positive");
  if (!img) return fail(T2O_EINVAL, "img is null");
  if (op == OP_DYNAMIC) {
    if (!op_id) return fail(T2O_EINVAL, "op_id is null");
    if (!param || param_stride < kMaxParam) return fail(T2O_EINVAL, "apply: param rows must be padded to >= 24 floats");
  } else {
    if (!op_supported(op)) return fail(T2O_EUNSUPPORTED, "operator index not supported (4 = inpaint needs EdgeConnect)");
    if (op >= 0 && op != OP_WHITE && (!param || param_stride < op_num_params(op)))
      return fail(T2O_EINVAL, "param is null or param_stride < number of operator parameters");
  }
  if ((mask == nullptr) != (mask_ch == 0) || !(mask_ch == 0 || mask_ch == 1 || mask_ch == 3))
    return fail(T2O_EINVAL, "mask_ch must be 0 (mask NULL), 1 or 3");
  if ((size_t)B * (size_t)sharp_num_tiles(H, W) > 0x7fffffffull || (size_t)H * W / 1 > 0x7fffffffull)
    return fail(T2O_EINVAL, "image too large for the launch grid");
  return T2O_OK;
}

int run_fwd(int op, const int* op_id, const float* img, const float* param, int param_stride, const float* mask,
            int mask_ch, const float* target, float* out, float* loss, void* ws, size_t ws_bytes, int B, int H, int W,
            void* stream) {
  if (int rc = check_common(op, op_id, img, param, param_stride, mask, mask_ch, B, H, W)) return rc;
  if (!out) return fail(T2O_EINVAL, "out is null");
  const Geometry g = launch_geometry(B, H, W);
  OpArgs a;
  memset(&a, 0, sizeof(a));
  a.img = img; a.param = param; a.mask = mask; a.op_id = op_id; a.target = target; a.out = out;
  a.op = op; a.param_stride = param_stride; a.mask_ch = mask_ch; a.B = B; a.H = H; a.W = W;
  a.iters = g.iters; a.nblk_max = g.nblk_max;
  a.inv_n = 1.0f / ((float)B * 3.0f * (float)H * (float)W);
  if (target) {
    if (!loss) return fail(T2O_EINVAL, "loss is null");
    if (!ws || ws_bytes < t2o_workspace_bytes(B, H, W)) return fail(T2O_EWORKSPACE, "workspace too small");
    a.loss_partials = (float*)ws + ws_partials_floats(g, B, H, W);
  }
  hipStream_t st = (hipStream_t)stream;
  if (op != OP_SHARPNESS) launch_point_fwd(a, g, st);
  if (op == OP_SHARPNESS || op == OP_DYNAMIC) launch_sharp_fwd(a, g, st);
  if (target) k_finalize_loss<<<1, kThreads, 0, st>>>(a, loss, g.nblk_point, sharp_fwd_blocks(a, g));
  return check_launch("operator forward");
}

int run_bwd(int op, const int* op_id, const float* img, const float* param, int param_stride, const float* mask,
            int mask_ch, const float* gout, const float* target, const float* gloss, float* gimg, float* gparam,
            int gparam_stride, void* ws, size_t ws_bytes, int B, int H, int W, void* stream,
            float* partials_region = nullptr, int* nblk_out = nullptr, float* value_out = nullptr, float* value_loss = nullptr) {
  if (int rc = check_common(op, op_id, img, param, param_stride, mask, mask_ch, B, H, W)) return rc;
  if (!target && !gout) return fail(T2O_EINVAL, "gout is null");
  if (target && !gloss) return fail(T2O_EINVAL, "gloss is null");
  if (!ws || ws_bytes < t2o_workspace_bytes(B, H, W)) return fail(T2O_EWORKSPACE, "workspace too small");
  if (gparam && gparam_stride < (op == OP_DYNAMIC ? kMaxParam : op_num_params(op)))
    return fail(T2O_EINVAL, "gparam_stride too small");
  Geometry g = launch_geometry(B, H, W);
  if (op == OP_COLOR || op == OP_TONE) {
    constexpr int mult = 4;
    const size_t groups = (size_t)H * W / g.vec;
    int it = g.iters * (mult > 0 ? mult : 1);
    if (it > 8) it = 8;
    g.iters = it;
    g.nblk_point = (int)((groups + (size_t)kThreads * it - 1) / ((size_t)kThreads * it));
  }
  OpArgs a;
  memset(&a, 0, sizeof(a));
  a.img = img; a.param = param; a.mask = mask; a.op_id = op_id; a.gout = gout; a.target = target; a.gloss = gloss;
  a.gimg = gimg; a.partials = partials_region ? partials_region : (float*)ws;
  a.op = op; a.param_stride = param_stride; a.mask_ch = mask_ch; a.B = B; a.H = H; a.W = W;
  a.iters = g.iters; a.nblk_max = g.nblk_max;
  a.inv_n = 1.0f / ((float)B * 3.0f * (float)H * (float)W);
  hipStream_t st = (hipStream_t)stream;
  if (value_loss) {
    if (op != OP_SHARPNESS || !target || mask_ch || !sharp_bwd_uses_strips(a, g)) return fail(T2O_EUNSUPPORTED, "value-and-gradient: unmasked sharpness on the strip kernels only");
    a.out = value_out;
    a.loss_partials = (float*)ws + ws_partials_floats(g, B, H, W);
  }
  if (partials_region) {
    if (op != OP_SHARPNESS) launch_point_bwd(a, g, st);
    else launch_sharp_bwd(a, g, st);
    if (nblk_out) *nblk_out = (op == OP_SHARPNESS) ? sharp_bwd_blocks(a, g) : g.nblk_point;
    return check_launch("operator backward");
  }
  if (op != OP_SHARPNESS) launch_point_bwd(a, g, st);
  if (op == OP_SHARPNESS || op == OP_DYNAMIC) launch_sharp_bwd(a, g, st);
  if (gparam && op != OP_IDENTITY)
    k_finalize_params<<<B, kThreads, 0, st>>>(a, gparam, gparam_stride, g.nblk_point, sharp_bwd_blocks(a, g));
  if (value_loss) k_finalize_loss<<<1, kThreads, 0, st>>>(a, value_loss, g.nblk_point, sharp_bwd_blocks(a, g));
  return check_launch("operator backward");
}

}

namespace {
__global__ __launch_bounds__(256) void k_zero_floats(float* p, size_t n) {
  const size_t i = (size_t)blockIdx.x * 256 + threadIdx.x;
  if (i < n) p[i] = 0.0f;
}
}

extern "C" {

int t2o_abi_version(void) { return 4; }
const char* t2o_last_error(void) { return g_err; }

int t2o_op_num_params(int op) { return (op >= 0 && op <= 7) ? op_num_params(op) : -1; }

size_t t2o_workspace_bytes(int B, int H, int W) {
  if (B <= 0 || H <= 0 || W <= 0) return 0;
  const Geometry g = launch_geometry(B, H, W);
  size_t f = ws_partials_floats(g, B, H, W) + ws_loss_floats(g, B, H, W);
  const size_t n = (size_t)B * 3 * H * W;
  const size_t l1blk = n / ((size_t)kThreads * 8) + 2;
  if (f < l1blk) f = l1blk;
  return f * sizeof(float);
}

int t2o_op_fwd(int op, const float* img, const float* param, int param_stride, const float* mask, int mask_ch,
               float* out, int B, int H, int W, void* stream) {
  if (op == OP_DYNAMIC) return fail(T2O_EUNSUPPORTED, "use t2o_apply_fwd for per-sample operators");
  return run_fwd(op, nullptr, img, param, param_stride, mask, mask_ch, nullptr, out, nullptr, nullptr, 0, B, H, W, stream);
}

int t2o_op_bwd(int op, const float* img, const float* param, int param_stride, const float* mask, int mask_ch,
               const float* gout, float* gimg, float* gparam, int gparam_stride, void* workspace,
               size_t workspace_bytes, int B, int H, int W, void* stream) {
  if (op == OP_DYNAMIC) return fail(T2O_EUNSUPPORTED, "use t2o_apply_bwd for per-sample operators");
  return run_bwd(op, nullptr, img, param, param_stride, mask, mask_ch, gout, nullptr, nullptr, gimg, gparam,
                 gparam_stride, workspace, workspace_bytes, B, H, W, stream);
}

int t2o_apply_fwd(const int* op_id, const float* img, const float* param, int param_stride, const float* mask,
                  int mask_ch, float* out, int B, int H, int W, void* stream) {
  return run_fwd(OP_DYNAMIC, op_id, img, param, param_stride, mask, mask_ch, nullptr, out, nullptr, nullptr, 0, B, H, W,
                 stream);
}

int t2o_apply_bwd(const int* op_id, const float* img, const float* param, int param_stride, const float* mask,
                  int mask_ch, const float* gout, float* gimg, float* gparam, int gparam_stride, void* workspace,
                  size_t workspace_bytes, int B, int H, int W, void* stream) {
  return run_bwd(OP_DYNAMIC, op_id, img, param, param_stride, mask, mask_ch, gout, nullptr, nullptr, gimg, gparam,
                 gparam_stride, workspace, workspace_bytes, B, H, W, stream);
}

int t2o_op_fwd_l1(int op, const float* img, const float* param, int param_stride, const float* mask, int mask_ch,
                  const float* target, float* out, float* loss, void* workspace, size_t workspace_bytes, int B, int H,
                  int W, void* stream) {
  if (!target) return fail(T2O_EINVAL, "target is null");
  if (op == OP_DYNAMIC) return fail(T2O_EUNSUPPORTED, "fused L1 takes a static operator");
  return run_fwd(op, nullptr, img, param, param_stride, mask, mask_ch, target, out, loss, workspace, workspace_bytes, B,
                 H, W, stream);
}

int t2o_op_bwd_l1(int op, const float* img, const float* param, int param_stride, const float* mask, int mask_ch,
                  const float* target, const float* gloss, float* gimg, float* gparam, int gparam_stride,
                  void* workspace, size_t workspace_bytes, int B, int H, int W, void* stream) {
  if (!target) return fail(T2O_EINVAL, "target is null");
  if (op == OP_DYNAMIC) return fail(T2O_EUNSUPPORTED, "fused L1 takes a static operator");
  return run_bwd(op, nullptr, img, param, param_stride, mask, mask_ch, nullptr, target, gloss, gimg, gparam,
                 gparam_stride, workspace, workspace_bytes, B, H, W, stream);
}

int t2o_l1_fwd(const float* pred, const float* target, float* loss, size_t n, void* workspace, size_t workspace_bytes,
               void* stream) {
  if (!pred || !target || !loss || n == 0) return fail(T2O_EINVAL, "l1_fwd: null pointer or n == 0");
  const int V = (n % 4 == 0) ? 4 : 1;
  const int iters = 8;
  const size_t groups = n / V;
  const size_t nblk = (groups + (size_t)kThreads * iters - 1) / ((size_t)kThreads * iters);
  if (!workspace || workspace_bytes < nblk * sizeof(float)) return fail(T2O_EWORKSPACE, "workspace too small");
  hipStream_t st = (hipStream_t)stream;
  float* partial = (float*)workspace;
  if (V == 4) k_l1_fwd<4><<<(unsigned)nblk, kThreads, 0, st>>>(pred, target, partial, n, iters);
  else k_l1_fwd<1><<<(unsigned)nblk, kThreads, 0, st>>>(pred, target, partial, n, iters);
  k_l1_finalize<<<1, kThreads, 0, st>>>(partial, (int)nblk, 1.0f / (float)n, loss);
  return check_launch("l1 forward");
}

int t2o_l1_bwd(const float* pred, const float* target, const float* gloss, float* gpred, size_t n, void* stream) {
  if (!pred || !target || !gloss || !gpred || n == 0) return fail(T2O_EINVAL, "l1_bwd: null pointer or n == 0");
  const int V = (n % 4 == 0) ? 4 : 1;
  const int iters = 4;
  const size_t groups = n / V;
  const size_t nblk = (groups + (size_t)kThreads * iters - 1) / ((size_t)kThreads * iters);
  hipStream_t st = (hipStream_t)stream;
  if (V == 4) k_l1_bwd<4><<<(unsigned)nblk, kThreads, 0, st>>>(pred, target, gloss, gpred, n, 1.0f / (float)n, iters);
  else k_l1_bwd<1><<<(unsigned)nblk, kThreads, 0, st>>>(pred, target, gloss, gpred, n, 1.0f / (float)n, iters);
  return check_launch("l1 backward");
}

int t2o_end_select_l1_fwd(const float* const* imgs, int T, const long long* first, const float* target, float* loss, int B,
                          size_t row, void* workspace, size_t workspace_bytes, void* stream) {
  if (!imgs || !first || !target || !loss || T < 1 || T > 8 || B <= 0 || row == 0) return fail(T2O_EINVAL, "end_select_l1_fwd: null pointer or bad shape (1 <= T <= 8)");
  EndSelArgs s = {};
  s.T = T;
  for (int t = 0; t < T; ++t) { if (!imgs[t]) return fail(T2O_EINVAL, "end_select_l1_fwd: null image"); s.img[t] = imgs[t]; }
  const size_t n = (size_t)B * row;
  const int V = (row % 4 == 0) ? 4 : 1;
  const int iters = 8;
  const size_t groups = n / V;
  const size_t nblk = (groups + (size_t)kThreads * iters - 1) / ((size_t)kThreads * iters);
  if (!workspace || workspace_bytes < nblk * sizeof(float)) return fail(T2O_EWORKSPACE, "workspace too small");
  hipStream_t st = (hipStream_t)stream;
  float* partial = (float*)workspace;
  if (V == 4) k_end_l1_fwd<4><<<(unsigned)nblk, kThreads, 0, st>>>(s, first, target, partial, n, row, iters);
  else k_end_l1_fwd<1><<<(unsigned)nblk, kThreads, 0, st>>>(s, first, target, partial, n, row, iters);
  k_l1_finalize<<<1, kThreads, 0, st>>>(partial, (int)nblk, 1.0f / (float)n, loss);
  return check_launch("END select + l1 forward");
}

int t2o_end_select_l1_bwd(const float* const* imgs, float* const* gimgs, int T, const long long* first, const float* target,
                          const float* gloss, int B, size_t row, void* stream) {
  if (!imgs || !gimgs || !first || !target || !gloss || T < 1 || T > 8 || B <= 0 || row == 0)
    return fail(T2O_EINVAL, "end_select_l1_bwd: null pointer or bad shape (1 <= T <= 8)");
  EndSelArgs s = {};
  s.T = T;
  for (int t = 0; t < T; ++t) {
    if (!imgs[t] || !gimgs[t]) return fail(T2O_EINVAL, "end_select_l1_bwd: null image");
    s.img[t] = imgs[t]; s.gimg[t] = gimgs[t];
  }
  const size_t n = (size_t)B * row;
  const int V = (row % 4 == 0) ? 4 : 1;
  const int iters = 4;
  const size_t groups = n / V;
  const size_t nblk = (groups + (size_t)kThreads * iters - 1) / ((size_t)kThreads * iters);
  hipStream_t st = (hipStream_t)stream;
  if (V == 4) k_end_l1_bwd<4><<<(unsigned)nblk, kThreads, 0, st>>>(s, first, target, gloss, n, row, 1.0f / (float)n, iters);
  else k_end_l1_bwd<1><<<(unsigned)nblk, kThreads, 0, st>>>(s, first, target, gloss, n, row, 1.0f / (float)n, iters);
  return check_launch("END select + l1 backward");
}

int t2o_sequence_fwd(const int* ops, int K, const float* img, const float* params, const float* target, float* acts,
                     float* loss, void* workspace, size_t workspace_bytes, int B, int H, int W, void* stream) {
  if (!ops || K <= 0 || !params || !acts) return fail(T2O_EINVAL, "sequence_fwd: null pointer or K <= 0");
  const size_t img_floats = (size_t)B * 3 * H * W;
  const float* cur = img;
  for (int k = 0; k < K; ++k) {
    float* out = acts + (size_t)k * img_floats;
    const float* p = params + (size_t)k * B * kMaxParam;
    const bool last = (k == K - 1) && target;
    const int rc = run_fwd(ops[k], nullptr, cur, p, kMaxParam, nullptr, 0, last ? target : nullptr, out,
                           last ? loss : nullptr, workspace, workspace_bytes, B, H, W, stream);
    if (rc) return rc;
    cur = out;
  }
  return T2O_OK;
}

int t2o_sequence_bwd(const int* ops, int K, const float* img, const float* params, const float* target,
                     const float* acts, const float* gloss, float* gimg, float* gparams, float* gbuf, void* workspace,
                     size_t workspace_bytes, int B, int H, int W, void* stream) {
  if (!ops || K <= 0 || !params || !acts || !target || !gloss || !gparams || !gbuf)
    return fail(T2O_EINVAL, "sequence_bwd: null pointer or K <= 0");
  if (!workspace || workspace_bytes < t2o_workspace_bytes(B, H, W)) return fail(T2O_EWORKSPACE, "workspace too small");
  const size_t img_floats = (size_t)B * 3 * H * W;
  const Geometry g = launch_geometry(B, H, W);
  const bool multi = K <= kMaxChain;
  const size_t region = (size_t)B * ws_block_rows(g, B, H, W) * kRedSlots;
  MultiFinalize mf;
  memset(&mf, 0, sizeof(mf));
  mf.params = params; mf.gparams = gparams; mf.partials = (const float*)workspace; mf.region_floats = region;
  mf.K = K; mf.B = B; mf.nblk_max = g.nblk_max;
  const float* gcur = nullptr;
  for (int k = K - 1; k >= 0; --k) {
    const float* in = k == 0 ? img : acts + (size_t)(k - 1) * img_floats;
    const float* p = params + (size_t)k * B * kMaxParam;
    float* gp = gparams + (size_t)k * B * kMaxParam;
    float* gout_next = (k == 0) ? gimg : gbuf + (size_t)(k & 1) * img_floats;
    const bool last = k == K - 1;
    float* reg = (multi && ops[k] != OP_IDENTITY) ? (float*)workspace + (size_t)k * region : nullptr;
    int nb = 0;
    const int rc = run_bwd(ops[k], nullptr, in, p, kMaxParam, nullptr, 0, last ? nullptr : gcur, last ? target : nullptr,
                           last ? gloss : nullptr, gout_next, gp, kMaxParam, workspace, workspace_bytes, B, H, W, stream,
                           reg, &nb);
    if (rc) return rc;
    if (multi) { mf.ops[k] = ops[k]; mf.nblk[k] = nb; }
    gcur = gout_next;
  }
  if (multi) {
    k_finalize_params_multi<<<(unsigned)(K * B), kThreads, 0, (hipStream_t)stream>>>(mf);
    return check_launch("sequence backward finalize");
  }
  return T2O_OK;
}

int t2o_fused_sequence_buffers(const int* ops, int K) {
  Segment seg[64];
  const int ns = plan_segments(ops, K, seg, 64);
  return ns < 0 ? -1 : ns - 1;
}

}

using SeqCfg2 = StaticChain<OP_BRIGHTNESS, OP_CONTRAST, OP_SATURATION, OP_COLOR, OP_TONE>;
using SeqCfg5 = StaticChain<OP_TONE, OP_COLOR, OP_TONE, OP_COLOR, OP_BRIGHTNESS, OP_CONTRAST, OP_SATURATION>;

template <class SEQ>
static bool chain_is(const ChainArgs& a) {
  if (a.K != SEQ::K) return false;
  for (int k = 0; k < SEQ::K; ++k)
    if (a.ops[k] != SEQ::ops[k]) return false;
  return true;
}
template <class SEQ, bool SV_LDS, int MINW>
static void launch_static_bwd(ChainArgs& a, bool l1, hipStream_t st) {
  const unsigned grid = (unsigned)a.B * a.nblk;
  const size_t lds = sizeof(float) * ((size_t)a.bin_off[kMaxChain] * kAccStride + (SV_LDS ? chain_save_floats<1>(SEQ::K) : 0));
  if (l1 && a.loss_partials) k_chain_bwd_static<true, SEQ, SV_LDS, MINW, true><<<grid, kThreads, lds, st>>>(a);
  else if (l1) k_chain_bwd_static<true, SEQ, SV_LDS, MINW><<<grid, kThreads, lds, st>>>(a);
  else k_chain_bwd_static<false, SEQ, SV_LDS, MINW><<<grid, kThreads, lds, st>>>(a);
}
template <class SEQ>
// ... 390 lines not shown
```

t2onet_amd/encoder.py:

```python
import os

import torch

from . import _lib
from .functional import (_need_gpu, _persistent_grad, _ptr, _stream, _conv_workspace, _zero_block, wino_conv_nhwc, wino_fused_conv_nhwc, wino_wgrad_nhwc, wino_input,
                         wino_backward_nhwc, wino_dw_from, wino_fused_wgrad_nhwc)

_WINOGRAD = os.environ.get('T2O_WINOGRAD', '1') != '0'
_WINO_MIN_C = int(os.environ.get('T2O_WINOGRAD_MIN_C', '256'))
_DUAL_BN = True
_WINO_FUSED = os.environ.get('T2O_WINOGRAD_FUSED', '1') != '0'
_BN_SUMS_EPILOGUE = True
_WINO_WGRAD = os.environ.get('T2O_WINOGRAD_WGRAD', '1') != '0'


def _fast_direct(stride, Hi, Wi, Wo):
    return Wo % 8 == 0 and (stride == 1 or (Hi % 2 == 0 and Wi % 2 == 0))


def _batched(fn, name, st, srcs, dsts, int_lists):
    import ctypes
    for i in range(0, len(srcs), 32):
        n = min(32, len(srcs) - i)
        a = (ctypes.c_void_p * n)(*[t.data_ptr() for t in srcs[i:i + n]])
        b = (ctypes.c_void_p * n)(*[t.data_ptr() for t in dsts[i:i + n]])
        ints = [(ctypes.c_int * n)(*lst[i:i + n]) for lst in int_lists]
        _lib.check(fn(a, b, *ints, n, st), name)


def _nhwc(N, H, W, C, dev):
    return torch.empty((N, H, W, C), dtype=torch.float32, device=dev)


class TrunkPlan:

    def __init__(self, resnet):
        self.net = resnet
        blocks = [b for layer in (resnet.layer1, resnet.layer2, resnet.layer3, resnet.layer4) for b in layer]
        self.blocks = blocks
        self.params = [resnet.conv1.weight, resnet.bn1.weight, resnet.bn1.bias]
        self.index = {}
        for b in blocks:
            self.params += [b.conv1.weight, b.bn1.weight, b.bn1.bias, b.conv2.weight, b.bn2.weight, b.bn2.bias]
            if len(b.shortcut):
                self.params += [b.shortcut[0].weight, b.shortcut[1].weight, b.shortcut[1].bias]
        for i, p in enumerate(self.params):
            self.index[id(p)] = i
        self.bns = [resnet.bn1] + [m for b in blocks for m in ([b.bn1, b.bn2] + ([b.shortcut[1]] if len(b.shortcut) else []))]
        self.pool = False
        self.persistent_wt = False
        self._wt = None
        self._wt_valid = False
        self._uf, self._uf_valid = None, False
        self._ub = {}

    def weights_changed(self):
        self._wt_valid = False
        self._uf_valid = False

    def _versions(self):
        return tuple(p._version for p in self.params if p.dim() == 4)

    def wino(self, conv, H, W):
        w = conv.weight
        return (_WINOGRAD and conv.stride[0] == 1 and H % 2 == 0 and W % 2 == 0 and w.shape[0] >= _WINO_MIN_C and w.shape[1] >= _WINO_MIN_C
                and w.shape[0] <= 1024 and w.shape[1] <= 1024 and (w.shape[0] & (w.shape[0] - 1)) == 0 and (w.shape[1] & (w.shape[1] - 1)) == 0
                and w.shape[0] % 128 == 0 and w.shape[1] % 128 == 0)

    def fused_wino(self, conv, H, W):
        w = conv.weight
        return (_WINO_FUSED and _WINOGRAD and conv.stride[0] == 1 and not self.wino(conv, H, W) and w.shape[0] in (64, 128)
                and w.shape[1] in (64, 128) and H % 16 == 0 and W % 16 == 0)

    def onchip_wgrad(self, conv, H, W):
        w = conv.weight
        return (_WINO_WGRAD and _WINO_FUSED and _WINOGRAD and conv.stride[0] == 1 and (self.fused_wino(conv, H, W) or self.wino(conv, H, W))
                and bool(_lib.load().t2o_wino_fused_wgrad_supported(1, H, W, w.shape[1], w.shape[0]))
                and bool(_lib.load().t2o_wino_fused_supported(1, H, W, w.shape[1], w.shape[0])))

    def kernel_for(self, conv, N, Hi, Wi, direction):
        key = (id(conv), N, Hi, Wi, direction, _WINOGRAD, _WINO_MIN_C, _WINO_FUSED, _WINO_WGRAD)
        memo = self.__dict__.setdefault('_kernel_memo', {})
        fam = memo.get(key)
        if fam is None:
            fam = memo[key] = self._kernel_for(conv, N, Hi, Wi, direction)
        return fam

    def _kernel_for(self, conv, N, Hi, Wi, direction):
        w = conv.weight
# ... 302 lines not shown

        def act_like(t, key):
            slot = arena.x_slot(key, apass) if apass is not None else None
            return slot if slot is not None else torch.empty_like(t)

        def conv3(x, conv, Nn, Hi, Wi, want_stats):
            w = conv.weight
            Co, Ci = w.shape[0], w.shape[1]
            s = conv.stride[0]
            Ho, Wo = (Hi - 1) // s + 1, (Wi - 1) // s + 1
            if plan.wino(conv, Hi, Wi):
                if plan.kernel_for(conv, Nn, Hi, Wi, 'wgrad') == 'wino_wgrad':
                    return wino_fused_conv_nhwc(x, uf[('c', id(conv))], Nn, Hi, Wi, None, True)
                keep = []
                y, stats = wino_conv_nhwc(x, uf[id(conv)], Nn, Hi, Wi, None, True, keep_v=keep,
                                          v_out=arena.wino_slot('V', conv, apass) if apass is not None else None,
                                          uc=uf.get(('c', id(conv))))
                kept_v[id(conv)] = keep[0]
                return y, stats
            fam = plan.kernel_for(conv, Nn, Hi, Wi, 'fwd')
            if fam == 'wino_fused':
                return wino_fused_conv_nhwc(x, uf[('c', id(conv))], Nn, Hi, Wi, None, True)
            y = _nhwc(Nn, Ho, Wo, Co, dev)
            if fam == 'direct':
                stats = torch.empty((lib.t2o_conv3x3_fwd_stats_rows(Nn, Ho, Wo, Co, s), 2, Co), dtype=torch.float32, device=dev)
                rc = lib.t2o_conv3x3_fwd_stats_nhwc(_ptr(x), _ptr(w), _ptr(y), _ptr(stats), _ptr(conv_ws), conv_ws.numel(), Nn, Ho, Wo,
                                                    Ci, Co, s, st)
                _lib.check(rc, 't2o_conv3x3_fwd_stats_nhwc')
                return y, stats
            _lib.check(lib.t2o_conv3x3_any_fwd_nhwc(_ptr(x), _ptr(w), _ptr(y), Nn, Hi, Wi, Ci, Co, s, st), 't2o_conv3x3_any_fwd_nhwc')
            return y, None

        Ho, Wo = H // 2, W // 2
        C0 = net.conv1.weight.shape[0]
        y0 = _nhwc(N, Ho, Wo, C0, dev)
        st0 = torch.empty((lib.t2o_stem_fwd_stats_rows(N, Ho, Wo), 2, C0), dtype=torch.float32, device=dev)
        _lib.check(lib.t2o_stem_fwd(_ptr(img), _ptr(net.conv1.weight), _ptr(y0), _ptr(st0), N, Ho, Wo, C0, planar, st), 't2o_stem_fwd')
        a0 = act_like(y0, 'a0')
        m0, i0 = _bn_fwd(lib, st, bn_ws, net.bn1, y0, a0, None, 1, st0, N * Ho * Wo, C0)
        stem = (y0, m0, i0)
        x, Hc, Wc = a0, Ho, Wo
        for bi, b in enumerate(plan.blocks):
            s = b.conv1.stride[0]
            Co = b.conv1.weight.shape[0]
            Hn, Wn = (Hc - 1) // s + 1, (Wc - 1) // s + 1
            M = N * Hn * Wn
            y1, s1 = conv3(x, b.conv1, N, Hc, Wc, True)
            a1 = act_like(y1, (bi, 'a1'))
            m1, i1 = _bn_fwd(lib, st, bn_ws, b.bn1, y1, a1, None, 1, s1, M, Co)
            rec = {'x': x, 'y1': y1, 'm1': m1, 'i1': i1, 'a1': a1, 'H': Hc, 'W': Wc}
            dual = bool(len(b.shortcut)) and _DUAL_BN
            if len(b.shortcut):
                sc_conv, sc_bn = b.shortcut[0], b.shortcut[1]
                ys = _nhwc(N, Hn, Wn, Co, dev)
                rc = lib.t2o_conv1x1s2_fwd_nhwc(_ptr(x), _ptr(sc_conv.weight), _ptr(ys), N, Hc, Wc, sc_conv.weight.shape[1], Co, st)
                _lib.check(rc, 't2o_conv1x1s2_fwd_nhwc')
                if not dual:
                    sc = torch.empty_like(ys)
                    ms, is_ = _bn_fwd(lib, st, bn_ws, sc_bn, ys, sc, None, 0, None, M, Co)
                    rec.update(ys=ys, ms=ms, is_=is_)
            else:
                sc = x
            y2, s2 = conv3(a1, b.conv2, N, Hn, Wn, True)
            out = act_like(y2, (bi, 'out'))
            if dual:
                m2, i2, ms, is_ = (torch.empty(Co, dtype=torch.float32, device=dev) for _ in range(4))
                need = lib.t2o_bn_dual_nhwc_workspace_bytes(M, Co)
                dws = torch.empty(need, dtype=torch.uint8, device=dev)
                rc = lib.t2o_bn_dual_relu_nhwc_fwd(_ptr(y2), _ptr(s2), 0 if s2 is None else s2.shape[0], _ptr(ys),
                                                   _ptr(b.bn2.weight), _ptr(b.bn2.bias), _ptr(b.bn2.running_mean), _ptr(b.bn2.running_var),
                                                   _ptr(m2), _ptr(i2), _ptr(sc_bn.weight), _ptr(sc_bn.bias), _ptr(sc_bn.running_mean),
                                                   _ptr(sc_bn.running_var), _ptr(ms), _ptr(is_), _ptr(out), float(b.bn2.momentum),
                                                   float(b.bn2.eps), float(sc_bn.momentum), float(sc_bn.eps), _ptr(dws), need, M, Co, st)
                _lib.check(rc, 't2o_bn_dual_relu_nhwc_fwd')
                rec.update(ys=ys, ms=ms, is_=is_, dual=True)
            else:
                m2, i2 = _bn_fwd(lib, st, bn_ws, b.bn2, y2, out, sc, 1, s2, M, Co)
            rec.update(y2=y2, m2=m2, i2=i2, out=out)
            saved.append(rec)
            x, Hc, Wc = out, Hn, Wn
        ctx.plan, ctx.img, ctx.stem, ctx.saved, ctx.planar = plan, img, stem, saved, planar
        ctx.a0 = a0
        ctx.kept_v = kept_v
        ctx.arena, ctx.apass = (arena, apass) if apass is not None else (None, None)
        ctx.into_grad = into_grad
        ctx.grads = [p.grad for p in plan.params] if ctx.into_grad else None
        ctx.pooled = plan.pool
        if plan.pool:
            ctx.hw = (x.shape[1], x.shape[2])
            return x.mean((1, 2))
        return x.permute(0, 3, 1, 2)

    @staticmethod
    def backward(ctx, dout):
        plan, net = ctx.plan, ctx.plan.net
        lib = _lib.load()
        dev = dout.device
        st = _stream(dev)
        acc = 1 if (ctx.into_grad and all(p.grad is g_ for p, g_ in zip(plan.params, ctx.grads))) else 0
        N = ctx.img.shape[0]
        grads = ctx.grads if acc else [torch.empty_like(p) for p in plan.params]

        def g(p):
            return grads[plan.index[id(p)]]

        bn_ws = torch.empty(lib.t2o_bn_nhwc_workspace_bytes(1, 512), dtype=torch.uint8, device=dev)
        conv_ws = _conv_workspace(dev, 64 << 10)
        wt = plan.transformed(lib, st)

        arena, apass = (ctx.arena, ctx.apass) if acc else (None, None)

        def deferred(conv):
            return arena.dy_slot(conv, apass) if arena is not None else None

        def bn_bwd(bn, x, y, dy, mean, invstd, has_res, relu, want_dres, M, C, dx=None):
            dx = torch.empty_like(x) if dx is None else dx
            dres = torch.empty_like(x) if want_dres else None
            rc = lib.t2o_bn_relu_nhwc_bwd_acc(_ptr(x), _ptr(y), _ptr(dy), _ptr(bn.weight), _ptr(bn.bias), _ptr(mean), _ptr(invstd),
                                              _ptr(dx), _ptr(dres), _ptr(g(bn.weight)), _ptr(g(bn.bias)), has_res, relu, acc,
                                              _ptr(bn_ws), bn_ws.numel(), M, C, st)
            _lib.check(rc, 't2o_bn_relu_nhwc_bwd_acc')
            return dx, dres

        def wgrad3(conv, x, dy, Hi, Wi, Hn, Wn):
            w = conv.weight
            Co, Ci = w.shape[0], w.shape[1]
            s = conv.stride[0]
            fam = plan.kernel_for(conv, N, Hi, Wi, 'wgrad')
            if fam == 'wino_wgrad':
                if not wino_fused_wgrad_nhwc(x, dy, g(w), N, Hi, Wi, bool(acc)):
                    raise RuntimeError('trunk: the on-chip Winograd weight gradient refused a layer the plan gave it')
                return
            if fam == 'wino_sep':
                V = ctx.kept_v.pop(id(conv), None)
                wino_wgrad_nhwc(V if V is not None else wino_input(x, N, Hi, Wi), dy, g(w), N, Hi, Wi, acc)
                return
            if fam == 'direct':
                need = (lib.t2o_conv3x3_wgrad_workspace_bytes if s == 1 else lib.t2o_conv3x3s2_wgrad_workspace_bytes)(N, Hn, Wn, Ci, Co)
                ws = torch.empty(need, dtype=torch.uint8, device=dev)
                rc = lib.t2o_conv3x3_wgrad_acc_nhwc(_ptr(x), _ptr(dy), _ptr(g(w)), _ptr(ws), need, N, Hn, Wn, Ci, Co, s, acc, st)
                _lib.check(rc, 't2o_conv3x3_wgrad_acc_nhwc')
                return
            need = lib.t2o_conv3x3_any_wgrad_workspace_bytes(N, Hi, Wi, Ci, Co, s)
            ws = torch.empty(need, dtype=torch.uint8, device=dev)
            rc = lib.t2o_conv3x3_any_wgrad_nhwc(_ptr(x), _ptr(dy), _ptr(g(w)), _ptr(ws), need, N, Hi, Wi, Ci, Co, s, acc, st)
            _lib.check(rc, 't2o_conv3x3_any_wgrad_nhwc')

        def wino_bwd(conv, x, dy, dx, addend, Hi, Wi):
            V = ctx.kept_v.pop(id(conv), None)
            if V is None:
                V = wino_input(x, N, Hi, Wi)
            ad_out = arena.wino_slot('Ad', conv, apass) if arena is not None else None
            wino_backward_nhwc(dy, V, wt['wino'][id(conv)], g(conv.weight), dx, N, Hi, Wi, addend, acc, ad_out,
                               uc=wt['wino'].get(('c', id(conv))))

        def dgrad3(conv, dy, dx, addend, Hi, Wi, Hn, Wn):
            w = conv.weight
            Co, Ci = w.shape[0], w.shape[1]
            s = conv.stride[0]
            fam = plan.kernel_for(conv, N, Hi, Wi, 'dgrad')
            if fam == 'wino_fused':
                wino_fused_conv_nhwc(dy, wt['wino'][('c', id(conv))], N, Hi, Wi, addend, False, out=dx)
                return
            if fam == 'wino_sep':
                wino_conv_nhwc(dy, wt['wino'][id(conv)], N, Hi, Wi, addend, False, out=dx)
                return
# ... 27 lines not shown
                slots = deferred(sc_conv)
                dy2 = slot2 if slot2 is not None else torch.empty_like(rec['y2'])
                dys = slots if slots is not None else torch.empty_like(rec['ys'])
                need = lib.t2o_bn_dual_nhwc_workspace_bytes(M, Co)
                dws = torch.empty(need, dtype=torch.uint8, device=dev)
                rc = lib.t2o_bn_dual_relu_nhwc_bwd_acc(_ptr(rec['y2']), _ptr(rec['ys']), _ptr(rec['out']), _ptr(d), _ptr(b.bn2.weight),
                                                       _ptr(b.bn2.bias), _ptr(rec['m2']), _ptr(rec['i2']), _ptr(sc_bn.weight), _ptr(sc_bn.bias),
                                                       _ptr(rec['ms']), _ptr(rec['is_']), _ptr(dy2), _ptr(dys), _ptr(g(b.bn2.weight)),
                                                       _ptr(g(b.bn2.bias)), _ptr(g(sc_bn.weight)), _ptr(g(sc_bn.bias)), acc, _ptr(dws), need,
                                                       M, Co, st)
                _lib.check(rc, 't2o_bn_dual_relu_nhwc_bwd_acc')
                dsc = None
            else:
                dy2, dsc = bn_bwd(b.bn2, rec['y2'], rec['out'], d, rec['m2'], rec['i2'], 1, 1, True, M, Co, slot2)
            da1 = torch.empty_like(rec['a1'])
            rows1 = None
            if plan.wino(b.conv2, Hn, Wn) and plan.kernel_for(b.conv2, N, Hn, Wn, 'wgrad') != 'wino_wgrad':
                wino_bwd(b.conv2, rec['a1'], dy2, da1, None, Hn, Wn)
            else:
                C2o, C2i = b.conv2.weight.shape[0], b.conv2.weight.shape[1]
                fam2 = plan.kernel_for(b.conv2, N, Hn, Wn, 'dgrad')
                fused2 = fam2 == 'wino_fused'
                n_rows = lib.t2o_conv3x3_dgrad_bnsums_rows(N, Hn, Wn, C2i, C2o) if (_BN_SUMS_EPILOGUE and fam2 == 'direct') else 0
                if fused2 and _BN_SUMS_EPILOGUE:
                    rows1 = torch.empty(lib.t2o_wino_fused_stats_rows(N, Hn, Wn) * 2 * C2i, dtype=torch.float32, device=dev)
                    rc = lib.t2o_wino_fused_conv_bnsums_nhwc(_ptr(dy2), _ptr(wt['wino'][('c', id(b.conv2))]), _ptr(da1), _ptr(rec['y1']),
                                                             _ptr(rec['m1']), _ptr(rec['i1']), _ptr(b.bn1.weight), _ptr(b.bn1.bias), _ptr(rows1),
                                                             _ptr(_zero_block(dev)), N, Hn, Wn, C2o, C2i, st)
                    _lib.check(rc, 't2o_wino_fused_conv_bnsums_nhwc')
                elif n_rows > 0:
                    rows1 = torch.empty(n_rows * 2 * C2i, dtype=torch.float32, device=dev)
                    rc = lib.t2o_conv3x3_dgrad_pre_bnsums_nhwc(_ptr(dy2), _ptr(wt[id(b.conv2)]), _ptr(da1), _ptr(rec['y1']), _ptr(rec['m1']),
                                                               _ptr(rec['i1']), _ptr(b.bn1.weight), _ptr(b.bn1.bias), _ptr(rows1),
                                                               _ptr(conv_ws), conv_ws.numel(), N, Hn, Wn, C2i, C2o, st)
                    _lib.check(rc, 't2o_conv3x3_dgrad_pre_bnsums_nhwc')
                else:
                    dgrad3(b.conv2, dy2, da1, None, Hn, Wn, Hn, Wn)
                if slot2 is None:
                    wgrad3(b.conv2, rec['a1'], dy2, Hn, Wn, Hn, Wn)
            del dy2
            slot1 = deferred(b.conv1)
            if rows1 is not None:
                dy1 = slot1 if slot1 is not None else torch.empty_like(rec['y1'])
                rc = lib.t2o_bn_relu_nhwc_bwd_partials_acc(_ptr(rec['y1']), _ptr(da1), _ptr(b.bn1.weight), _ptr(b.bn1.bias), _ptr(rec['m1']),
                                                           _ptr(rec['i1']), _ptr(dy1), _ptr(g(b.bn1.weight)), _ptr(g(b.bn1.bias)), 1, acc,
                                                           _ptr(rows1), rows1.numel() // (2 * Co), _ptr(bn_ws), bn_ws.numel(), M, Co, st)
                _lib.check(rc, 't2o_bn_relu_nhwc_bwd_partials_acc')
            else:
                dy1, _ = bn_bwd(b.bn1, rec['y1'], None, da1, rec['m1'], rec['i1'], 0, 1, False, M, Co, slot1)
            del da1
            dx = torch.empty_like(rec['x'])
            if plan.wino(b.conv1, Hc, Wc) and not len(b.shortcut) and plan.kernel_for(b.conv1, N, Hc, Wc, 'wgrad') != 'wino_wgrad':
                wino_bwd(b.conv1, rec['x'], dy1, dx, dsc, Hc, Wc)
                d = dx
                continue
            if slot1 is None:
                wgrad3(b.conv1, rec['x'], dy1, Hc, Wc, Hn, Wn)
            if len(b.shortcut):
                sc_conv, sc_bn = b.shortcut[0], b.shortcut[1]
                if dys is None:
                    slots = deferred(sc_conv)
                    dys, _ = bn_bwd(sc_bn, rec['ys'], None, dsc, rec['ms'], rec['is_'], 0, 0, False, M, Co, slots)
                if slots is None:
                    need = lib.t2o_conv1x1s2_wgrad_workspace_bytes(N, Hc, Wc, Ci, Co)
                    ws = torch.empty(need, dtype=torch.uint8, device=dev)
                    rc = lib.t2o_conv1x1s2_wgrad_nhwc(_ptr(rec['x']), _ptr(dys), _ptr(g(sc_conv.weight)), _ptr(ws), need, N, Hc, Wc, Ci, Co,
                                                      acc, st)
                    _lib.check(rc, 't2o_conv1x1s2_wgrad_nhwc')
                dgrad3(b.conv1, dy1, dx, None, Hc, Wc, Hn, Wn)
                rc = lib.t2o_conv1x1s2_dgrad_acc_nhwc(_ptr(dys), _ptr(wt[id(sc_conv)]), _ptr(dx), N, Hc, Wc, Ci, Co, st)
                _lib.check(rc, 't2o_conv1x1s2_dgrad_acc_nhwc')
            else:
                dgrad3(b.conv1, dy1, dx, dsc, Hc, Wc, Hn, Wn)
            d = dx
        y0, m0, i0 = ctx.stem
        _, Ho, Wo, C0 = y0.shape
        dy0, _ = bn_bwd(net.bn1, y0, None, d, m0, i0, 0, 1, False, N * Ho * Wo, C0)
        need = lib.t2o_stem_wgrad_workspace_bytes(N, Ho, Wo, C0)
        ws = torch.empty(need, dtype=torch.uint8, device=dev)
        rc = lib.t2o_stem_wgrad(_ptr(ctx.img), _ptr(dy0), _ptr(g(net.conv1.weight)), _ptr(ws), need, N, Ho, Wo, C0, ctx.planar, acc, st)
        _lib.check(rc, 't2o_stem_wgrad')
        dimg = None
        if ctx.needs_input_grad[1]:
            dimg = torch.empty_like(ctx.img)
            rc = lib.t2o_stem_dgrad(_ptr(dy0), _ptr(net.conv1.weight), _ptr(dimg), N, Ho, Wo, C0, ctx.planar, 0, st)
            _lib.check(rc, 't2o_stem_dgrad')
        if arena is not None:
            arena.done.add(apass)
        return (None, dimg) + (tuple(None for _ in plan.params) if acc else tuple(grads))


def trunk_forward(plan, img, pool=False):
    plan.pool = bool(pool)
    return _TrunkFn.apply(plan, img, *plan.params)
```

t2onet_amd/functional.py:

```python
import ctypes

import os

import numpy as np
import torch

from . import _lib

OP_NPARAM = (1, 1, 1, 24, 1, 8, 1, 1)
PARAM_PAD = 24
_workspaces = {}


_raw_stream = getattr(torch._C, '_cuda_getCurrentRawStream', None)


def _stream(device=None):
    if _raw_stream is not None:
        return _raw_stream(torch.cuda.current_device() if device is None or device.index is None else device.index)
    return torch.cuda.current_stream(device).cuda_stream


def _ptr(t):
    return None if t is None else t.data_ptr()


def _need_gpu(*ts):
    for t in ts:
        if t is not None and not (t.is_cuda and t.dtype == torch.float32):
            raise RuntimeError('t2onet_amd: expected fp32 tensors on the GPU (got %s on %s); '
                               'there is no CPU implementation' % (t.dtype, t.device))


def _img(t):
    if t.dim() != 4 or t.shape[1] != 3:
        raise ValueError('image must be (B,3,H,W), got %s' % (tuple(t.shape),))
    return t.contiguous()


def _mask(mask, img):
    if mask is None:
        return None, 0
    B, _, H, W = img.shape
    if mask.dim() != 4 or mask.shape[0] != B or mask.shape[1] not in (1, 3) or tuple(mask.shape[2:]) != (H, W):
        mask = mask.expand(B, mask.shape[1] if mask.shape[1] in (1, 3) else 3, H, W)
    return mask.contiguous(), mask.shape[1]


_ws_need = {}


def _scratch(need, device):
    if torch.cuda.is_current_stream_capturing():
        return torch.empty(max(need, 1 << 20), dtype=torch.uint8, device=device)
    key = (device.index, _stream(device))
    ws = _workspaces.get(key)
    if ws is None or ws.numel() < need:
        ws = torch.empty(max(need, 1 << 20), dtype=torch.uint8, device=device)
        _workspaces[key] = ws
    return ws


def workspace(B, H, W, device):
    need = _ws_need.get((B, H, W))
    if need is None:
        need = _ws_need[(B, H, W)] = _lib.load().t2o_workspace_bytes(B, H, W)
    return _scratch(need, device)


class _OperatorFn(torch.autograd.Function):

    @staticmethod
    def forward(ctx, img, param, mask, op):
        _need_gpu(img, param, mask)
        img = _img(img)
        param = param.contiguous()
        mask, mask_ch = _mask(mask, img)
        B, _, H, W = img.shape
        out = torch.empty_like(img)
        rc = _lib.load().t2o_op_fwd(op, _ptr(img), _ptr(param), param.shape[1], _ptr(mask), mask_ch, _ptr(out),
                                    B, H, W, _stream(img.device))
        _lib.check(rc, 't2o_op_fwd')
        ctx.save_for_backward(img, param, mask)
        ctx.op, ctx.mask_ch = op, mask_ch
        return out

    @staticmethod
    def backward(ctx, gout):
        img, param, mask = ctx.saved_tensors
        B, _, H, W = img.shape
        gout = gout.contiguous()
        gimg = torch.empty_like(img) if ctx.needs_input_grad[0] else None
        gparam = torch.empty_like(param) if ctx.op in (0, 1, 2, 3, 5, 6) and param.shape[1] == OP_NPARAM[ctx.op] \
            else torch.zeros_like(param)
        ws = workspace(B, H, W, img.device)
        rc = _lib.load().t2o_op_bwd(ctx.op, _ptr(img), _ptr(param), param.shape[1], _ptr(mask), ctx.mask_ch,
                                    _ptr(gout), _ptr(gimg), _ptr(gparam), gparam.shape[1], _ptr(ws), ws.numel(),
                                    B, H, W, _stream(img.device))
        _lib.check(rc, 't2o_op_bwd')
        return gimg, gparam, None, None


def operator_apply(op, img, param, mask=None):
    return _OperatorFn.apply(img, param, mask, int(op))


class _ApplyFn(torch.autograd.Function):

    @staticmethod
    def forward(ctx, img, param, mask, op_id):
        _need_gpu(img, param, mask)
        if op_id.dtype != torch.int32 or not op_id.is_cuda:
            raise RuntimeError('op_id must be an int32 GPU tensor')
        img = _img(img)
        param = param.contiguous()
        op_id = op_id.contiguous()
        mask, mask_ch = _mask(mask, img)
        B, _, H, W = img.shape
        if param.shape != (B, PARAM_PAD):
            raise ValueError('param must be (B,24)')
        out = torch.empty_like(img)
        rc = _lib.load().t2o_apply_fwd(_ptr(op_id), _ptr(img), _ptr(param), PARAM_PAD, _ptr(mask), mask_ch,
                                       _ptr(out), B, H, W, _stream(img.device))
        _lib.check(rc, 't2o_apply_fwd')
        ctx.save_for_backward(img, param, mask, op_id)
        ctx.mask_ch = mask_ch
        return out

    @staticmethod
    def backward(ctx, gout):
        img, param, mask, op_id = ctx.saved_tensors
        B, _, H, W = img.shape
        gout = gout.contiguous()
        gimg = torch.empty_like(img) if ctx.needs_input_grad[0] else None
        gparam = torch.zeros_like(param)
        ws = workspace(B, H, W, img.device)
        rc = _lib.load().t2o_apply_bwd(_ptr(op_id), _ptr(img), _ptr(param), PARAM_PAD, _ptr(mask), ctx.mask_ch,
                                       _ptr(gout), _ptr(gimg), _ptr(gparam), PARAM_PAD, _ptr(ws), ws.numel(),
                                       B, H, W, _stream(img.device))
        _lib.check(rc, 't2o_apply_bwd')
        return gimg, gparam, None, None


def apply_per_sample(op_id, img, param, mask=None):
    return _ApplyFn.apply(img, param, mask, op_id)


class _L1Fn(torch.autograd.Function):
    @staticmethod
    def forward(ctx, pred, target):
        _need_gpu(pred, target)
        pred, target = pred.contiguous(), target.contiguous()
        if pred.shape != target.shape:
            raise ValueError('l1_loss: shape mismatch')
        loss = torch.empty((), dtype=torch.float32, device=pred.device)
        n = pred.numel()
        ws = workspace(max(1, n // (3 * 64 * 64) + 1), 64, 64, pred.device)
        rc = _lib.load().t2o_l1_fwd(_ptr(pred), _ptr(target), _ptr(loss), n, _ptr(ws), ws.numel(), _stream(pred.device))
        _lib.check(rc, 't2o_l1_fwd')
        ctx.save_for_backward(pred, target)
        return loss

    @staticmethod
    def backward(ctx, gloss):
        pred, target = ctx.saved_tensors
        gloss = gloss.contiguous().to(torch.float32)
        gpred = torch.empty_like(pred)
        rc = _lib.load().t2o_l1_bwd(_ptr(pred), _ptr(target), _ptr(gloss), _ptr(gpred), pred.numel(), _stream(pred.device))
        _lib.check(rc, 't2o_l1_bwd')
        return gpred, None


def l1_loss(pred, target):
    return _L1Fn.apply(pred, target)


def _ptr_array(tensors):
    return (ctypes.c_void_p * len(tensors))(*[t.data_ptr() for t in tensors])


class _EndSelectL1Fn(torch.autograd.Function):

    @staticmethod
    def forward(ctx, first, target, *imgs):
        _need_gpu(target, *imgs)
        imgs = [t.contiguous() for t in imgs]
        target = target.contiguous()
        if any(t.shape != target.shape for t in imgs):
            raise ValueError('end_select_l1: shape mismatch')
        B = target.shape[0]
        row = target.numel() // B
        first = first.to(torch.int64).contiguous()
        loss = torch.empty((), dtype=torch.float32, device=target.device)
        n = target.numel()
        ws = workspace(max(1, n // (3 * 64 * 64) + 1), 64, 64, target.device)
        rc = _lib.load().t2o_end_select_l1_fwd(_ptr_array(imgs), len(imgs), _ptr(first), _ptr(target), _ptr(loss), B, row, _ptr(ws),
                                               ws.numel(), _stream(target.device))
        _lib.check(rc, 't2o_end_select_l1_fwd')
        ctx.save_for_backward(first, target, *imgs)
        return loss

    @staticmethod
    def backward(ctx, gloss):
        first, target = ctx.saved_tensors[:2]
        imgs = list(ctx.saved_tensors[2:])
        gloss = gloss.contiguous().to(torch.float32)
        grads = [torch.empty_like(t) for t in imgs]
        B = target.shape[0]
        rc = _lib.load().t2o_end_select_l1_bwd(_ptr_array(imgs), _ptr_array(grads), len(imgs), _ptr(first), _ptr(target), _ptr(gloss), B,
                                               target.numel() // B, _stream(target.device))
        _lib.check(rc, 't2o_end_select_l1_bwd')
        return (None, None) + tuple(grads)


def end_select_l1(imgs, first, target):
    return _EndSelectL1Fn.apply(first, target, *imgs)


class _AttnFn(torch.autograd.Function):
    @staticmethod
    def forward(ctx, q, context):
        _need_gpu(q, context)
        q, context = q.contiguous(), context.contiguous()
        B, L, D = context.shape
        attn = torch.empty(B, L, dtype=torch.float32, device=q.device)
        mix = torch.empty(B, D, dtype=torch.float32, device=q.device)
        rc = _lib.load().t2o_attn_fwd(_ptr(q), _ptr(context), _ptr(attn), _ptr(mix), B, L, D, _stream(q.device))
        _lib.check(rc, 't2o_attn_fwd')
        ctx.save_for_backward(q, context, attn)
        return mix, attn

    @staticmethod
    def backward(ctx, gmix, gattn):
        q, context, attn = ctx.saved_tensors
        B, L, D = context.shape
        gmix = gmix.contiguous()
        gattn = None if gattn is None else gattn.contiguous()
        gq = torch.empty_like(q)
        gctx = torch.empty_like(context)
        rc = _lib.load().t2o_attn_bwd(_ptr(q), _ptr(context), _ptr(attn), _ptr(gmix), _ptr(gattn), _ptr(gq),
                                      _ptr(gctx), B, L, D, _stream(q.device))
        _lib.check(rc, 't2o_attn_bwd')
        return gq, gctx


def attention_core(q, context):
    return _AttnFn.apply(q, context)


def choose_op(logp, op_mask, explore_prob, sample=True, u=None):
    _need_gpu(logp, op_mask)
    B, n = op_mask.shape
    logp = logp.detach().reshape(B, n).contiguous()
    if not op_mask.is_contiguous():
        raise ValueError('choose_op: op_mask must be contiguous (it is updated in place)')
    if not sample:
        u = None
    elif u is None:
        u = torch.rand(B, device=logp.device, dtype=torch.float32)
    pred = torch.empty(B, 1, dtype=torch.int64, device=logp.device)
    exe = torch.empty(B, dtype=torch.int32, device=logp.device)
    rc = _lib.load().t2o_choose_op(_ptr(logp), _ptr(op_mask), _ptr(u), float(explore_prob), _ptr(pred), _ptr(exe), B, n, _stream(logp.device))
    _lib.check(rc, 't2o_choose_op')
    return pred, exe


def _is_nhwc(x):
    C = x.shape[1]
    return (x.dim() == 4 and C >= 4 and C <= 1024 and (C & (C - 1)) == 0 and x.shape[2] * x.shape[3] > 1
            and x.is_contiguous(memory_format=torch.channels_last))


class _BnReluFn(torch.autograd.Function):

    @staticmethod
    def forward(ctx, x, res, weight, bias, running_mean, running_var, momentum, eps, relu=True, partial=None):
        _need_gpu(x, res, weight, bias)
        nhwc = _is_nhwc(x)
        if not relu and not nhwc:
            raise RuntimeError('batch norm without the activation is only built for channels-last activations')
        fmt = torch.channels_last if nhwc else torch.contiguous_format
        x = x.contiguous(memory_format=fmt)
        res = None if res is None else res.contiguous(memory_format=fmt)
        N, C = x.shape[0], x.shape[1]
        HW = x.numel() // (N * C)
        lib = _lib.load()
        out = torch.empty_like(x)
        save_mean = torch.empty(C, dtype=torch.float32, device=x.device)
        save_invstd = torch.empty(C, dtype=torch.float32, device=x.device)
        ws = _bn_workspace(lib, N, C, x.device, nhwc, HW)
        if nhwc and partial is not None:
# ... 1703 lines not shown
```

t2onet_amd/train.py:

```python
import os

import torch
import torch.distributed as dist
import torch.nn.functional as F

from . import functional as T


def first_end_step(pred_ops, end_id):
    B, Tn = pred_ops.shape
    is_end = pred_ops == end_id
    return torch.where(is_end.any(1), is_end.int().argmax(1), torch.full((B,), Tn - 1, device=pred_ops.device))


def select_end_images(pred_imgs, pred_ops, end_id):
    first = first_end_step(pred_ops, end_id)
    return pred_imgs[torch.arange(pred_ops.shape[0], device=pred_ops.device), first]


def end_l1_loss(pred_imgs, pred_ops, end_id, target):
    if target.is_cuda and target.dtype == torch.float32 and 1 <= len(pred_imgs) <= 8:
        return T.end_select_l1(pred_imgs, first_end_step(pred_ops, end_id), target)
    return T.l1_loss(select_end_images(torch.stack(pred_imgs, 1), pred_ops, end_id), target)

# ... 150 lines not shown
        if 'offsets' in sd:
            src_off, src_n = list(sd['offsets']), list(sd['numels'])
        else:
            src_n, src_off, n = numels, [], 0
            for k in numels:
                src_off.append(n)
                n += k
        if src_n != numels:
            raise ValueError('FlatAdam.load_state_dict: the saved state belongs to other parameters (%d tensors / %d elements, this '
                             'model has %d / %d)' % (len(src_n), sum(src_n), len(numels), sum(numels)))
        need = src_off[-1] + src_n[-1] if src_n else 0
        for name in ('exp_avg', 'exp_avg_sq'):
            if sd[name].numel() < need:
                raise ValueError('FlatAdam.load_state_dict: %s holds %d elements, its layout needs %d' % (name, sd[name].numel(), need))
        self.step_count = int(sd['step'])
        for name, dst in (('exp_avg', self.exp_avg), ('exp_avg_sq', self.exp_avg_sq)):
            src = sd[name].reshape(-1)
            if src_off == list(self.grads.offsets) and src.numel() == dst.numel():
                dst.copy_(src)
            else:
                dst.zero_()
                for so, do, k in zip(src_off, self.grads.offsets, numels):
                    dst[do:do + k].copy_(src[so:so + k])
        self.lr, self.betas, self.eps = float(sd['lr']), tuple(sd['betas']), float(sd['eps'])


class Trainer:

    def __init__(self, model, opt, lr=None, graph_encoder=False, graph_step=False):
        self.model, self.opt = model, opt
        self.grads = FlatGradients(model.parameters())
        lr = lr if lr is not None else opt.learning_rate
        if self.grads.flat.is_cuda:
            self.optimizer = FlatAdam(self.grads, lr=lr)
        else:
            self.optimizer = torch.optim.Adam(self.grads.params, lr=lr)
        self.itr = 0
        self.graph_encoder = graph_encoder
        self.graph_step = graph_step
        self._step_graphs = {}
        self.max_step_graphs = 4
        enc = getattr(model, 'vis_encoder', None)
        self._trunk = enc.trunk_plan() if (enc is not None and self.grads.flat.is_cuda and hasattr(enc, 'trunk_plan')) else None
        if self._trunk is not None:
            self._trunk.persistent_wt = True
        executor = getattr(model, 'executor', None)
        if executor is not None and self.grads.flat.is_cuda:
            executor.__dict__['heads_grad_in_place'] = True
        self._tape_owner = model if (self.grads.flat.is_cuda and hasattr(model, 'decoder') and hasattr(model, 'bn1')) else None

    def close(self):
        self.grads.close()

    def _tape(self, B):
        model = self._tape_owner
        if model is None:
            return None
        tape = self.__dict__.get('_tape_obj')
        if tape is None or tape.B != B:
            from .decoder_step import DecoderTape
            dec = model.decoder
            tape = self._tape_obj = DecoderTape(B, dec.hidden_size, dec.word_vec_dim, dec.output_size, model.vis_encoder.fc.in_features,
                                                self.opt.decoder_max_len + 1, self.grads.flat.device, persistent=True)
        model.__dict__['_tape'] = model.decoder.__dict__['_tape'] = tape
        tape.begin()
        return tape

    def _flush_tape(self):
        model = self._tape_owner
        tape = model.__dict__.get('_tape') if model is not None else None
        if tape is not None:
            tape.flush(model)
        arena = self._trunk.__dict__.get('arena') if self._trunk is not None else None
        if arena is not None:
            arena.flush(self._trunk)

    def _release(self):
        model = self._tape_owner
        if model is not None:
            model.__dict__.pop('_tape', None)
            model.decoder.__dict__.pop('_tape', None)
        if self._trunk is not None:
            self._trunk.__dict__['arena'] = None

    MAX_ARENAS = 2

    def _arena(self, img, passes):
        if self._trunk is None or self.graph_encoder or not img.is_cuda:
            return
        key = (img.shape[0], img.shape[2], img.shape[3])
        arenas = self.__dict__.setdefault('_arenas', {})
        arena = arenas.pop(key, None)
        if passes <= 0 or not self._trunk.supported(img):
            if arena is not None:
                arenas[key] = arena
            self._trunk.__dict__['arena'] = None
            return
        if arena is not None and arena.P < passes:
            arena = None
        if arena is None:
            from .encoder import WgradArena
            while len(arenas) >= self.MAX_ARENAS:
                arenas.pop(next(iter(arenas)))
            arena = WgradArena(self._trunk, key[0], key[1], key[2], passes, img.device)
        arenas[key] = arena
        self._trunk.__dict__['arena'] = arena
        arena.begin()

    def _maybe_graph(self, img):
        if self.graph_encoder and img.is_cuda and '_graphed_encoders' not in self.model.__dict__:
            self.model.train()
            try:
                self.model.graph_image_encoder(img, self.opt.decoder_max_len + 1)
            except Exception as e:
                import warnings
                warnings.warn('image-encoder graph capture failed (%s: %s); continuing without it' % (type(e).__name__, e))
                self.graph_encoder = False

    def _finish(self, loss):
        self.grads.zero()
        loss.backward()
        self._flush_tape()
        self._update()

    def _update(self):
        self.grads.all_reduce_mean()
        self.optimizer.step()
        if self._trunk is not None:
            self._trunk.weights_changed()

    def _request_length(self, x, lengths):
        if not self.model.variable_lengths:
            return int(x.shape[1])
        if lengths is not None and not (torch.is_tensor(lengths) and lengths.is_cuda):
            return int(max(lengths)) if not torch.is_tensor(lengths) else int(lengths.max())
        return int((x != self.opt.null_id).sum(1).max())

    def _graphed_episode_step(self, x, img_x, target, reinforce_sample, lengths):
        model = self.model
        if not (img_x.is_cuda and model.training and self.opt.decoder_max_len > 0):
            return None
        if lengths is None:
            lengths = (x != self.opt.null_id).sum(1)
        L = self._request_length(x, lengths)
        key = (tuple(img_x.shape), tuple(x.shape), L, bool(reinforce_sample))
        sg = self._step_graphs.get(key)
        if sg is None:
            if len(self._step_graphs) >= self.max_step_graphs:
                return None
            from .graphs import GraphedEpisodeStep
            try:
                sg = GraphedEpisodeStep(self, x, lengths, L, img_x, target, reinforce_sample)
            except Exception as e:
                import warnings
                warnings.warn('episode-step graph capture failed (%s: %s); continuing without it' % (type(e).__name__, e))
                self.graph_step = False
                return None
            self._step_graphs[key] = sg
            if self._trunk is not None:
                self._trunk.weights_changed()
        loss = sg.run(x, img_x, target)
        self._update()
        return loss

    def supervised_step(self, x, y, img_x, img_y, gt_params, lengths=None):
        step = int((y != self.opt.null_id).sum(1).max())
        self._maybe_graph(img_x)
        try:
            self._tape(img_x.shape[0])
            self._arena(img_x, step - 1)
            _, pred_params, logp = self.model.supervised_forward(x, y, img_x, img_y, gt_params, None, lengths)
            target = y[:, 1:step].contiguous().view(-1)
            op_loss = F.nll_loss(logp.reshape(-1, logp.shape[-1]), target)
            gt = gt_params[:, :step - 2]
            param_loss = F.mse_loss(pred_params, gt, reduction='sum') / ((gt != 0).sum())
            self._finish(op_loss + param_loss)
        finally:
            self._release()
        return op_loss.detach(), param_loss.detach()

    def episode_step(self, x, img_x, target, reinforce_sample=1, lengths=None):
        if self.graph_step:
            loss = self._graphed_episode_step(x, img_x, target, reinforce_sample, lengths)
            if loss is not None:
                return loss
        self._maybe_graph(img_x)
        try:
            self._tape(img_x.shape[0])
            self._arena(img_x, self.opt.decoder_max_len)
            _, pred_imgs, pred_ops, _ = self.model.episode_forward(x, img_x, None, reinforce_sample, lengths, stack=False)
            loss = end_l1_loss(pred_imgs, pred_ops, self.opt.end_id, target)
            self._finish(loss)
        finally:
            self._release()
        return loss.detach()

    def step(self, batch):
        self.itr += 1
        img_x, img_y, x, y, gt_params = batch
        if self.itr % 2 == 1:
            return self.supervised_step(x, y, img_x, img_y, gt_params)
        return self.episode_step(x, img_x, img_y[:, -1])
```

Before: 1857 images/sec.

## Fold END-select L1 gradient into apply backward and relay stem dgrad accumulation

Adds a gradient relay that, during the episode step, skips materialising separate END-select L1 gradient tensors for images consumed once by an apply op. Instead, the sign(x-t) term is added inside the apply backward kernels (pointwise and sharpness strips). The apply's input gradient can also be parked and handed to the encoder stem dgrad, which accumulates into it instead of writing a fresh tensor. The goal is to cut full-image gradient writes and autograd accumulation adds, at the cost of pointer-identity bookkeeping and forcing dynamic-op kernel variants on the chained path.

```diff
diff --git a/include/t2onet_hip.h b/include/t2onet_hip.h
--- a/include/t2onet_hip.h
+++ b/include/t2onet_hip.h
@@ -38,6 +38,11 @@
                   const float* mask, int mask_ch, const float* gout,
                   float* gimg, float* gparam, int gparam_stride,
                   void* workspace, size_t workspace_bytes, int B, int H, int W, void* stream);
+int t2o_apply_bwd_chain(const int* op_id, const float* img, const float* param, int param_stride,
+                        const float* mask, int mask_ch, const float* gout,
+                        const long long* end_first, const float* end_target, const float* end_gloss, int end_k,
+                        float* gimg, float* gparam, int gparam_stride,
+                        void* workspace, size_t workspace_bytes, int B, int H, int W, void* stream);
 
 int t2o_l1_fwd(const float* pred, const float* target, float* loss, size_t n,
                void* workspace, size_t workspace_bytes, void* stream);
@@ -48,6 +53,8 @@
                           size_t row, void* workspace, size_t workspace_bytes, void* stream);
 int t2o_end_select_l1_bwd(const float* const* imgs, float* const* gimgs, int T, const long long* first, const float* target,
                           const float* gloss, int B, size_t row, void* stream);
+int t2o_end_select_l1_bwd_one(const float* img, float* gimg, int k, const long long* first, const float* target,
+                              const float* gloss, int B, size_t row, void* stream);
 
 int t2o_op_fwd_l1(int op, const float* img, const float* param, int param_stride,
                   const float* mask, int mask_ch, const float* target, float* out, float* loss,
diff --git a/t2onet_amd/_lib.py b/t2onet_amd/_lib.py
--- a/t2onet_amd/_lib.py
+++ b/t2onet_amd/_lib.py
@@ -24,6 +24,7 @@
     't2o_op_bwd': (_I, [_I, _P, _P, _I, _P, _I, _P, _P, _P, _I, _P, _Z, _I, _I, _I, _P]),
     't2o_apply_fwd': (_I, [_P, _P, _P, _I, _P, _I, _P, _I, _I, _I, _P]),
     't2o_apply_bwd': (_I, [_P, _P, _P, _I, _P, _I, _P, _P, _P, _I, _P, _Z, _I, _I, _I, _P]),
+    't2o_apply_bwd_chain': (_I, [_P, _P, _P, _I, _P, _I, _P, _P, _P, _P, _I, _P, _P, _I, _P, _Z, _I, _I, _I, _P]),
     't2o_l1_fwd': (_I, [_P, _P, _P, _Z, _P, _Z, _P]),
     't2o_l1_bwd': (_I, [_P, _P, _P, _P, _Z, _P]),
     't2o_op_fwd_l1': (_I, [_I, _P, _P, _I, _P, _I, _P, _P, _P, _P, _Z, _I, _I, _I, _P]),
@@ -100,6 +101,7 @@
     't2o_wino_weight_transform_chunked_batch': (_I, [_P, _P, _P, _P, _I, _P]),
     't2o_end_select_l1_fwd': (_I, [_P, _I, _P, _P, _P, _I, _Z, _P, _Z, _P]),
     't2o_end_select_l1_bwd': (_I, [_P, _P, _I, _P, _P, _P, _I, _Z, _P]),
+    't2o_end_select_l1_bwd_one': (_I, [_P, _P, _I, _P, _P, _P, _I, _Z, _P]),
     't2o_wino_padded_tiles': (_I, [_I, _I, _I]),
     't2o_wino_weight_transform': (_I, [_P, _P, _I, _I, _P]),
     't2o_gemm_nt_batched': (_I, [_P, _P, _P, _I, _I, _I, _I, _I, _P]),
diff --git a/t2onet_amd/csrc/t2o_block_programs.h b/t2onet_amd/csrc/t2o_block_programs.h
--- a/t2onet_amd/csrc/t2o_block_programs.h
+++ b/t2onet_amd/csrc/t2o_block_programs.h
@@ -39,6 +39,11 @@
   int iters;
   int nblk_max;
   float inv_n;
+  const float* end_target;
+  const long long* end_first;
+  const float* end_gloss;
+  int end_k;
+  float end_inv_n;
 };
 
 T2O_HD size_t plane_off(const OpArgs& a, int b, int c) { return ((size_t)b * 3 + c) * (size_t)a.H * a.W; }
@@ -74,6 +79,35 @@
 }
 
 T2O_HD float sign_of(float d) { return d > 0.0f ? 1.0f : (d < 0.0f ? -1.0f : 0.0f); }
+
+T2O_HD float add_rn(float a, float b) {
+#if defined(__HIP_DEVICE_COMPILE__)
+  return __fadd_rn(a, b);
+#else
+  return a + b;
+#endif
+}
+
+struct EndTerm { bool sel; float gs; };
+T2O_HD EndTerm end_term_of(const OpArgs& a, int b) {
+  EndTerm e;
+  e.sel = (int)a.end_first[b] == a.end_k;
+  e.gs = a.end_gloss[0] * a.end_inv_n;
+  return e;
+}
+template <int V>
+T2O_HD void end_add(const EndTerm& e, const float* img, const float* target, float (&g)[V]) {
+  if (e.sel) {
+    float x[V], t[V];
+    load_vec<V>(img, x);
+    load_vec<V>(target, t);
+    T2O_UNROLL
+    for (int i = 0; i < V; ++i) g[i] = add_rn(g[i], sign_of(x[i] - t[i]) * e.gs);
+  } else {
+    T2O_UNROLL
+    for (int i = 0; i < V; ++i) g[i] = add_rn(g[i], 0.0f);
+  }
+}
 
 constexpr int kTabStride = 64;
 constexpr int kTabK = 0, kTabP = 24, kTabSum = 51, kTabScale = 54, kTabRsum = 57;
@@ -192,7 +226,7 @@
   return l1;
 }
 
-template <int V, bool MASKED, bool L1>
+template <int V, bool MASKED, bool L1, bool END = false>
 T2O_HD void pointwise_bwd_thread(const OpArgs& a, int op, int b, int blk, int tid, float (&red)[kRedSlots], const float* tab) {
   const unsigned hw = (unsigned)a.H * (unsigned)a.W;
   const unsigned groups = hw / V;
@@ -207,6 +241,8 @@
   Curve cv;
   float p0[1] = {(op >= 0 && prow) ? prow[0] : 0.0f};
   const float gs = L1 ? a.gloss[0] * a.inv_n : 0.0f;
+  EndTerm et = {false, 0.0f};
+  if (END) et = end_term_of(a, b);
   for (int it = 0; it < a.iters; ++it) {
     const unsigned g = ((unsigned)blk * a.iters + it) * kThreads + tid;
     if (g >= groups) break;
@@ -272,6 +308,10 @@
     }
     }
     if (s.o) {
+      if (END) {
+        T2O_UNROLL
+        for (int c = 0; c < 3; ++c) end_add<V>(et, s.x + c * hw + px, a.end_target + sb + c * hw + px, gx[c]);
+      }
       T2O_UNROLL
       for (int c = 0; c < 3; ++c) store_vec<V>(s.o + c * hw + px, gx[c]);
     }
@@ -533,6 +573,18 @@
     }
     if (!live) continue;
     float* dst = a.gimg + plane_off(a, b, c) + (size_t)gy * a.W + gx0;
+    if (a.end_target) {
+      const EndTerm et = end_term_of(a, b);
+      const size_t off = plane_off(a, b, c) + (size_t)gy * a.W + gx0;
+      if (V == 4) end_add<4>(et, a.img + off, a.end_target + off, o);
+      else {
+        for (int i = 0; i < 4 && gx0 + i < a.W; ++i) {
+          float o1[1] = {o[i]};
+          end_add<1>(et, a.img + off + i, a.end_target + off + i, o1);
+          o[i] = o1[0];
+        }
+      }
+    }
     if (V == 4) store_vec<4>(dst, o);
     else for (int i = 0; i < 4 && gx0 + i < a.W; ++i) dst[i] = o[i];
   }
diff --git a/t2onet_amd/csrc/t2o_kernels.hip b/t2onet_amd/csrc/t2o_kernels.hip
--- a/t2onet_amd/csrc/t2o_kernels.hip
+++ b/t2onet_amd/csrc/t2o_kernels.hip
@@ -46,7 +46,7 @@
   if (L1) block_reduce_store1(l1, a.loss_partials + (size_t)b * a.nblk_max + blk);
 }
 
-template <int OP, int V, bool MASKED, bool L1>
+template <int OP, int V, bool MASKED, bool L1, bool END = false>
 __global__ __launch_bounds__(kThreads) void k_point_bwd(OpArgs a, int nblk) {
   int b, blk;
   wg_coords(nblk, b, blk);
@@ -63,14 +63,14 @@
   }
   if (OP == OP_DYNAMIC) {
     switch (op) {
-#define T2O_CASE(K) case K: pointwise_bwd_thread<V, MASKED, L1>(a, K, b, blk, threadIdx.x, red, tab); break;
+#define T2O_CASE(K) case K: pointwise_bwd_thread<V, MASKED, L1, END>(a, K, b, blk, threadIdx.x, red, tab); break;
       T2O_CASE(OP_BRIGHTNESS) T2O_CASE(OP_CONTRAST) T2O_CASE(OP_SATURATION) T2O_CASE(OP_COLOR)
       T2O_CASE(OP_TONE) T2O_CASE(OP_WHITE)
 #undef T2O_CASE
-      default: pointwise_bwd_thread<V, MASKED, L1>(a, OP_IDENTITY, b, blk, threadIdx.x, red, tab); break;
+      default: pointwise_bwd_thread<V, MASKED, L1, END>(a, OP_IDENTITY, b, blk, threadIdx.x, red, tab); break;
     }
   } else {
-    pointwise_bwd_thread<V, MASKED, L1>(a, OP, b, blk, threadIdx.x, red, tab);
+    pointwise_bwd_thread<V, MASKED, L1, END>(a, OP, b, blk, threadIdx.x, red, tab);
   }
   if (op == OP_IDENTITY || op == OP_WHITE) return;
   block_reduce_store(red, nred_of(op), a.partials + ((size_t)b * a.nblk_max + blk) * kRedSlots);
@@ -161,7 +161,7 @@
 }
 
 
-template <bool DYN, bool WIDE, bool MASKED, bool VAL = false>
+template <bool DYN, bool WIDE, bool MASKED, bool VAL = false, bool END = false>
 __global__ __launch_bounds__(kThreads) void k_sharp_bwd_strip(OpArgs a, int nblk, int nseg) {
   int b, blk;
   wg_coords(nblk, b, blk);
@@ -176,6 +176,8 @@
   const float gs = a.target ? a.gloss[0] * a.inv_n : 0.0f;
   float red0 = 0.0f;
   float l1 = 0.0f;
+  EndTerm et = {false, 0.0f};
+  if constexpr (END) et = end_term_of(a, b);
 #pragma unroll 1
   for (int c = 0; c < 3; ++c) {
     const float* xp = a.img + ((size_t)b * 3 + c) * hw;
@@ -239,8 +241,11 @@
         o[i] = ce[i] + p * sharp_delta(ce[i], g[k - 1][i], left, right, g[k + 1][i]);
         if (MASKED) o[i] = pass[k - 1][i] + o[i];
       }
-      if (a.gimg && own && col_live && y < a.H)
-        store_vec<4>(a.gimg + ((size_t)b * 3 + c) * hw + (unsigned)y * (unsigned)a.W + (unsigned)gx0, o);
+      if (a.gimg && own && col_live && y < a.H) {
+        const size_t off = ((size_t)b * 3 + c) * hw + (unsigned)y * (unsigned)a.W + (unsigned)gx0;
+        if constexpr (END) end_add<4>(et, a.img + off, a.end_target + off, o);
+        store_vec<4>(a.gimg + off, o);
+      }
     }
   }
   block_reduce_store1(red0, a.partials + ((size_t)b * a.nblk_max + blk) * kRedSlots);
@@ -527,6 +532,28 @@
 #pragma unroll
     for (int k = 0; k < 8; ++k)
       if (k < s.T) store_vec<V>(s.gimg[k] + g * V, f == k ? o : z);
+  }
+}
+
+template <int V>
+__global__ __launch_bounds__(kThreads) void k_end_l1_bwd_one(const float* img, float* gimg, int k, const long long* first,
+                                                             const float* target, const float* gloss, size_t n, size_t row,
+                                                             float inv_n, int iters) {
+  const float gs = gloss[0] * inv_n;
+  for (int it = 0; it < iters; ++it) {
+    const size_t g = ((size_t)blockIdx.x * iters + it) * kThreads + threadIdx.x;
+    if (g * V >= n) break;
+    float o[V];
+#pragma unroll
+    for (int i = 0; i < V; ++i) o[i] = 0.0f;
+    if ((int)first[(g * V) / row] == k) {
+      float p[V], t[V];
+      load_vec<V>(img + g * V, p);
+      load_vec<V>(target + g * V, t);
+#pragma unroll
+      for (int i = 0; i < V; ++i) o[i] = sign_of(p[i] - t[i]) * gs;
+    }
+    store_vec<V>(gimg + g * V, o);
   }
 }
 
@@ -937,6 +964,16 @@
   const int op = a.op, nblk = g.nblk_point;
   const bool masked = a.mask_ch != 0, l1 = a.target != nullptr;
   const unsigned grid = (unsigned)a.B * nblk;
+  if (a.end_target) {
+    if (g.vec == 4) {
+      if (masked) k_point_bwd<OP_DYNAMIC, 4, true, false, true><<<grid, kThreads, 0, st>>>(a, nblk);
+      else k_point_bwd<OP_DYNAMIC, 4, false, false, true><<<grid, kThreads, 0, st>>>(a, nblk);
+    } else {
+      if (masked) k_point_bwd<OP_DYNAMIC, 1, true, false, true><<<grid, kThreads, 0, st>>>(a, nblk);
+      else k_point_bwd<OP_DYNAMIC, 1, false, false, true><<<grid, kThreads, 0, st>>>(a, nblk);
+    }
+    return;
+  }
   if (g.vec == 4) { T2O_POINT_CASES(k_point_bwd, 4) } else { T2O_POINT_CASES(k_point_bwd, 1) }
 }
 bool sharp_uses_strips(const Geometry& g) {
@@ -981,6 +1018,14 @@
 #define T2O_BWD_STRIP(D, Wd) \
     { if (a.mask_ch) k_sharp_bwd_strip<D, Wd, true><<<grid, kThreads, 0, st>>>(a, nblk, nseg); \
       else k_sharp_bwd_strip<D, Wd, false><<<grid, kThreads, 0, st>>>(a, nblk, nseg); }
+#define T2O_BWD_STRIP_END(Wd) \
+    { if (a.mask_ch) k_sharp_bwd_strip<true, Wd, true, false, true><<<grid, kThreads, 0, st>>>(a, nblk, nseg); \
+      else k_sharp_bwd_strip<true, Wd, false, false, true><<<grid, kThreads, 0, st>>>(a, nblk, nseg); }
+    if (a.end_target) {
+      if (nseg > 1) T2O_BWD_STRIP_END(true) else T2O_BWD_STRIP_END(false)
+      return;
+    }
+#undef T2O_BWD_STRIP_END
     if (nseg > 1) { if (dyn) T2O_BWD_STRIP(true, true) else T2O_BWD_STRIP(false, true) }
     else          { if (dyn) T2O_BWD_STRIP(true, false) else T2O_BWD_STRIP(false, false) }
 #undef T2O_BWD_STRIP
@@ -1041,10 +1086,13 @@
   return check_launch("operator forward");
 }
 
+struct EndChain { const long long* first; const float* target; const float* gloss; int k; };
+
 int run_bwd(int op, const int* op_id, const float* img, const float* param, int param_stride, const float* mask,
             int mask_ch, const float* gout, const float* target, const float* gloss, float* gimg, float* gparam,
             int gparam_stride, void* ws, size_t ws_bytes, int B, int H, int W, void* stream,
-            float* partials_region = nullptr, int* nblk_out = nullptr, float* value_out = nullptr, float* value_loss = nullptr) {
+            float* partials_region = nullptr, int* nblk_out = nullptr, float* value_out = nullptr, float* value_loss = nullptr,
+            const EndChain* end = nullptr) {
   if (int rc = check_common(op, op_id, img, param, param_stride, mask, mask_ch, B, H, W)) return rc;
   if (!target && !gout) return fail(T2O_EINVAL, "gout is null");
   if (target && !gloss) return fail(T2O_EINVAL, "gloss is null");
@@ -1068,6 +1116,11 @@
   a.iters = g.iters; a.nblk_max = g.nblk_max;
   a.inv_n = 1.0f / ((float)B * 3.0f * (float)H * (float)W);
   hipStream_t st = (hipStream_t)stream;
+  if (end) {
+    if (op != OP_DYNAMIC || target || partials_region || value_loss || !gimg) return fail(T2O_EINVAL, "chained backward: per-sample operators with gout and gimg only");
+    a.end_target = end->target; a.end_first = end->first; a.end_gloss = end->gloss; a.end_k = end->k;
+    a.end_inv_n = 1.0f / (float)((size_t)B * 3 * (size_t)H * (size_t)W);
+  }
   if (value_loss) {
     if (op != OP_SHARPNESS || !target || mask_ch || !sharp_bwd_uses_strips(a, g)) return fail(T2O_EUNSUPPORTED, "value-and-gradient: unmasked sharpness on the strip kernels only");
     a.out = value_out;
@@ -1138,6 +1191,19 @@
                   size_t workspace_bytes, int B, int H, int W, void* stream) {
   return run_bwd(OP_DYNAMIC, op_id, img, param, param_stride, mask, mask_ch, gout, nullptr, nullptr, gimg, gparam,
                  gparam_stride, workspace, workspace_bytes, B, H, W, stream);
+}
+
+int t2o_apply_bwd_chain(const int* op_id, const float* img, const float* param, int param_stride, const float* mask,
+                        int mask_ch, const float* gout, const long long* end_first, const float* end_target,
+                        const float* end_gloss, int end_k, float* gimg, float* gparam, int gparam_stride, void* workspace,
+                        size_t workspace_bytes, int B, int H, int W, void* stream) {
+  if (!end_target)
+    return run_bwd(OP_DYNAMIC, op_id, img, param, param_stride, mask, mask_ch, gout, nullptr, nullptr, gimg, gparam,
+                   gparam_stride, workspace, workspace_bytes, B, H, W, stream);
+  if (!end_first || !end_gloss || end_k < 0 || end_k > 7) return fail(T2O_EINVAL, "apply_bwd_chain: END term needs first, gloss and 0 <= end_k <= 7");
+  const EndChain end = {end_first, end_target, end_gloss, end_k};
+  return run_bwd(OP_DYNAMIC, op_id, img, param, param_stride, mask, mask_ch, gout, nullptr, nullptr, gimg, gparam,
+                 gparam_stride, workspace, workspace_bytes, B, H, W, stream, nullptr, nullptr, nullptr, nullptr, &end);
 }
 
 int t2o_op_fwd_l1(int op, const float* img, const float* param, int param_stride, const float* mask, int mask_ch,
@@ -1225,6 +1291,21 @@
   if (V == 4) k_end_l1_bwd<4><<<(unsigned)nblk, kThreads, 0, st>>>(s, first, target, gloss, n, row, 1.0f / (float)n, iters);
   else k_end_l1_bwd<1><<<(unsigned)nblk, kThreads, 0, st>>>(s, first, target, gloss, n, row, 1.0f / (float)n, iters);
   return check_launch("END select + l1 backward");
+}
+
+int t2o_end_select_l1_bwd_one(const float* img, float* gimg, int k, const long long* first, const float* target,
+                              const float* gloss, int B, size_t row, void* stream) {
+  if (!img || !gimg || !first || !target || !gloss || k < 0 || k > 7 || B <= 0 || row == 0)
+    return fail(T2O_EINVAL, "end_select_l1_bwd_one: null pointer or bad shape (0 <= k <= 7)");
+  const size_t n = (size_t)B * row;
+  const int V = (row % 4 == 0) ? 4 : 1;
+  const int iters = 4;
+  const size_t groups = n / V;
+  const size_t nblk = (groups + (size_t)kThreads * iters - 1) / ((size_t)kThreads * iters);
+  hipStream_t st = (hipStream_t)stream;
+  if (V == 4) k_end_l1_bwd_one<4><<<(unsigned)nblk, kThreads, 0, st>>>(img, gimg, k, first, target, gloss, n, row, 1.0f / (float)n, iters);
+  else k_end_l1_bwd_one<1><<<(unsigned)nblk, kThreads, 0, st>>>(img, gimg, k, first, target, gloss, n, row, 1.0f / (float)n, iters);
+  return check_launch("END select + l1 backward (one image)");
 }
 
 int t2o_sequence_fwd(const int* ops, int K, const float* img, const float* params, const float* target, float* acts,
diff --git a/t2onet_amd/encoder.py b/t2onet_amd/encoder.py
--- a/t2onet_amd/encoder.py
+++ b/t2onet_amd/encoder.py
@@ -4,7 +4,7 @@
 
 from . import _lib
 from .functional import (_need_gpu, _persistent_grad, _ptr, _stream, _conv_workspace, _zero_block, wino_conv_nhwc, wino_fused_conv_nhwc, wino_wgrad_nhwc, wino_input,
-                         wino_backward_nhwc, wino_dw_from, wino_fused_wgrad_nhwc)
+                         wino_backward_nhwc, wino_dw_from, wino_fused_wgrad_nhwc, grad_relay)
 
 _WINOGRAD = os.environ.get('T2O_WINOGRAD', '1') != '0'
 _WINO_MIN_C = int(os.environ.get('T2O_WINOGRAD_MIN_C', '256'))
@@ -473,6 +473,9 @@
         ctx.plan, ctx.img, ctx.stem, ctx.saved, ctx.planar = plan, img, stem, saved, planar
         ctx.a0 = a0
         ctx.kept_v = kept_v
+        ctx.relay = grad_relay() if (ctx.needs_input_grad[1] and planar) else None
+        if ctx.relay is not None:
+            ctx.relay.saw(ctx.relay.trunk_imgs, img)
         ctx.arena, ctx.apass = (arena, apass) if apass is not None else (None, None)
         ctx.into_grad = into_grad
         ctx.grads = [p.grad for p in plan.params] if ctx.into_grad else None
@@ -666,8 +669,12 @@
         _lib.check(rc, 't2o_stem_wgrad')
         dimg = None
         if ctx.needs_input_grad[1]:
-            dimg = torch.empty_like(ctx.img)
-            rc = lib.t2o_stem_dgrad(_ptr(dy0), _ptr(net.conv1.weight), _ptr(dimg), N, Ho, Wo, C0, ctx.planar, 0, st)
+            relay = ctx.relay if ctx.relay is grad_relay() else None
+            dimg = relay.take(ctx.img) if relay is not None else None
+            into = 0 if dimg is None else 1
+            if dimg is None:
+                dimg = torch.empty_like(ctx.img)
+            rc = lib.t2o_stem_dgrad(_ptr(dy0), _ptr(net.conv1.weight), _ptr(dimg), N, Ho, Wo, C0, ctx.planar, into, st)
             _lib.check(rc, 't2o_stem_dgrad')
         if arena is not None:
             arena.done.add(apass)
diff --git a/t2onet_amd/functional.py b/t2onet_amd/functional.py
--- a/t2onet_amd/functional.py
+++ b/t2onet_amd/functional.py
@@ -103,6 +103,47 @@
 
 def operator_apply(op, img, param, mask=None):
     return _OperatorFn.apply(img, param, mask, int(op))
+
+
+_GRAD_RELAY = True
+
+
+class GradRelay:
+
+    def __init__(self):
+        self.begin()
+
+    def begin(self):
+        self.apply_imgs, self.trunk_imgs = {}, {}
+        self.end = None
+        self.parked = {}
+
+    def saw(self, table, img):
+        table[img.data_ptr()] = table.get(img.data_ptr(), 0) + 1
+
+    def end_chained(self, img):
+        return self.apply_imgs.get(img.data_ptr()) == 1
+
+    def wants_park(self, img):
+        return self.trunk_imgs.get(img.data_ptr()) == 1
+
+    def take(self, img):
+        g = self.parked.pop(img.data_ptr(), None)
+        self.trunk_imgs.pop(img.data_ptr(), None)
+        return g
+
+
+_relay = None
+
+
+def install_grad_relay(on=True):
+    global _relay
+    _relay = GradRelay() if (on and _GRAD_RELAY and not torch.cuda.is_current_stream_capturing()) else None
+    return _relay
+
+
+def grad_relay():
+    return _relay
 
 
 class _ApplyFn(torch.autograd.Function):
@@ -125,6 +166,9 @@
         _lib.check(rc, 't2o_apply_fwd')
         ctx.save_for_backward(img, param, mask, op_id)
         ctx.mask_ch = mask_ch
+        ctx.relay = _relay if ctx.needs_input_grad[0] else None
+        if ctx.relay is not None:
+            ctx.relay.saw(ctx.relay.apply_imgs, img)
         return out
 
     @staticmethod
@@ -135,6 +179,19 @@
         gimg = torch.empty_like(img) if ctx.needs_input_grad[0] else None
         gparam = torch.zeros_like(param)
         ws = workspace(B, H, W, img.device)
+        relay = ctx.relay if ctx.relay is _relay else None
+        if relay is not None and relay.apply_imgs.pop(img.data_ptr(), 0) == 1:
+            end = relay.end if (relay.end is not None and img.data_ptr() in relay.end[3]) else None
+            first, target, gloss, steps = end if end is not None else (None, None, None, {})
+            rc = _lib.load().t2o_apply_bwd_chain(_ptr(op_id), _ptr(img), _ptr(param), PARAM_PAD, _ptr(mask), ctx.mask_ch,
+                                                 _ptr(gout), _ptr(first), _ptr(target), _ptr(gloss), steps.get(img.data_ptr(), 0),
+                                                 _ptr(gimg), _ptr(gparam), PARAM_PAD, _ptr(ws), ws.numel(), B, H, W,
+                                                 _stream(img.device))
+            _lib.check(rc, 't2o_apply_bwd_chain')
+            if relay.wants_park(img):
+                relay.parked[img.data_ptr()] = gimg
+                gimg = None
+            return gimg, gparam, None, None
         rc = _lib.load().t2o_apply_bwd(_ptr(op_id), _ptr(img), _ptr(param), PARAM_PAD, _ptr(mask), ctx.mask_ch,
                                        _ptr(gout), _ptr(gimg), _ptr(gparam), PARAM_PAD, _ptr(ws), ws.numel(),
                                        B, H, W, _stream(img.device))
@@ -205,8 +262,24 @@
         first, target = ctx.saved_tensors[:2]
         imgs = list(ctx.saved_tensors[2:])
         gloss = gloss.contiguous().to(torch.float32)
+        B = target.shape[0]
+        relay = _relay
+        if relay is not None and relay.end is None and len(imgs) <= 8:
+            ptrs = [t.data_ptr() for t in imgs]
+            relay.end = (first, target, gloss, {p: k for k, (p, t) in enumerate(zip(ptrs, imgs))
+                                                if relay.end_chained(t) and ptrs.count(p) == 1})
+            grads = []
+            for k, t in enumerate(imgs):
+                if t.data_ptr() in relay.end[3] or not ctx.needs_input_grad[2 + k]:
+                    grads.append(None)
+                    continue
+                g = torch.empty_like(t)
+                rc = _lib.load().t2o_end_select_l1_bwd_one(_ptr(t), _ptr(g), k, _ptr(first), _ptr(target), _ptr(gloss), B,
+                                                           target.numel() // B, _stream(target.device))
+                _lib.check(rc, 't2o_end_select_l1_bwd_one')
+                grads.append(g)
+            return (None, None) + tuple(grads)
         grads = [torch.empty_like(t) for t in imgs]
-        B = target.shape[0]
         rc = _lib.load().t2o_end_select_l1_bwd(_ptr_array(imgs), _ptr_array(grads), len(imgs), _ptr(first), _ptr(target), _ptr(gloss), B,
                                                target.numel() // B, _stream(target.device))
         _lib.check(rc, 't2o_end_select_l1_bwd')
diff --git a/t2onet_amd/train.py b/t2onet_amd/train.py
--- a/t2onet_amd/train.py
+++ b/t2onet_amd/train.py
@@ -256,6 +256,7 @@
             model.decoder.__dict__.pop('_tape', None)
         if self._trunk is not None:
             self._trunk.__dict__['arena'] = None
+        T.install_grad_relay(False)
 
     MAX_ARENAS = 2
 
@@ -362,6 +363,8 @@
         try:
             self._tape(img_x.shape[0])
             self._arena(img_x, self.opt.decoder_max_len)
+            if img_x.is_cuda:
+                T.install_grad_relay()
             _, pred_imgs, pred_ops, _ = self.model.episode_forward(x, img_x, None, reinforce_sample, lengths, stack=False)
             loss = end_l1_loss(pred_imgs, pred_ops, self.opt.end_id, target)
             self._finish(loss)
```

After: 1867 images/sec (median of 6 runs). No clear change (+0.6%).
